# ZulutionAI/MoviiGen1.1

Measured on AMD Instinct MI355X. Metric: denoise-steps/sec, higher is better.
Workload: dtype bf16; 1 GPU; 14B T2V 1920x832x81f bf16 (the metric's configuration; BASELINE configs[2] shape); layers=40, parallelism=single, solver=unipc, weights=random N(0,0.02) bf16, seed 0

## Files before the change

### include/moviigen_hip.h

```cpp
#ifndef MOVIIGEN_HIP_H
#define MOVIIGEN_HIP_H

#include <stdint.h>

#ifdef __cplusplus
extern "C" {
#endif

#define MG_OK 0
#define MG_ERR_ARG (-1)
#define MG_ERR_SHAPE (-2)
#define MG_ERR_LAUNCH (-3)
#define MG_ERR_UNAVAILABLE (-4)
#define MG_ERR_COMM (-5)

const char* mg_version(void);
int mg_abi_version(void);


int mg_ln_modulate(const float* x, int64_t ldx, int64_t rows, int dim, const float* scale,
                   const float* shift, int add_one, float eps, int round_norm_bf16, void* out,
                   int out_f32, int64_t ldo, void* stream);

int64_t mg_step_resid_partials_bytes(void);
int mg_step_resid_capture_f32(float* r, const float* x, const float* xin, int64_t n, double* stats, double* partials,
                              void* stream);
int mg_resid_ln_modulate_f32(const float* x, int64_t ldx, const float* r, int64_t ldr, int64_t rows, int dim,
                             const float* scale, const float* shift, float eps, float* out, int64_t ldo, void* stream);

int mg_rmsnorm_rope_bf16(const uint16_t* x, int64_t ldx, uint16_t* out, int64_t ldo,
                         int64_t rows, int dim, const float* weight, float eps, int head_dim,
                         const float* rope_cs, int F, int H, int W, int64_t pos0, float out_scale, void* stream);

int mg_pack_kv_bf16(const uint16_t* k, int64_t ldk, const uint16_t* v, int64_t ldv, int64_t L,
                    int heads, int head_dim, uint16_t* kp, uint16_t* vp, void* stream);


enum {
    MG_EPI_BIAS_BF16 = 0,
    MG_EPI_BIAS_GELU_BF16 = 1,
    MG_EPI_GATE_RESID_F32 = 2,
    MG_EPI_BIAS_F32 = 3
};

int mg_gemm_bf16(const uint16_t* A, int64_t lda, const uint16_t* W, int64_t ldw,
                 const float* bias, int64_t M, int N, int K, int epilogue, void* out,
                 int64_t ldo, const float* gate, void* stream);

int mg_quant_mxfp8_rows(const uint16_t* x, int64_t ldx, int64_t rows, int K, uint8_t* q, int64_t ldq,
                        uint8_t* scales, int64_t lds, void* stream);

int mg_gemm_mxfp8(const uint8_t* Aq, int64_t lda, const uint8_t* As, int64_t ldas, const uint8_t* Wq, int64_t ldw,
                  const uint8_t* Ws, int64_t ldws, const float* bias, int64_t M, int N, int K, int epilogue,
                  void* out, int64_t ldo, const float* gate, void* stream);

int mg_ln_modulate_mxfp8(const float* x, int64_t ldx, int64_t rows, int dim, const float* scale, const float* shift,
                         int add_one, float eps, int round_norm_bf16, uint16_t* out, int64_t ldo, uint8_t* q,
                         int64_t ldq, uint8_t* scales, int64_t lds, void* stream);

int mg_gemm_mxfp8_gelu_q(const uint8_t* Aq, int64_t lda, const uint8_t* As, int64_t ldas, const uint8_t* Wq, int64_t ldw,
                         const uint8_t* Ws, int64_t ldws, const float* bias, int64_t M, int N, int K, uint8_t* oq,
                         int64_t ldoq, uint8_t* oscales, int64_t ldos, void* stream);

int64_t mg_attn_workspace_bytes(void);
int mg_attn_fwd_bf16_hd128(const uint16_t* q, int64_t ldq, const uint16_t* kp, const uint16_t* vp,
                           uint16_t* o, int64_t ldo, int64_t Lq, int64_t Lk, int heads, float scale,
                           void* workspace, void* stream);

int mg_attn_fwd_bf16_hd128_lse(const uint16_t* q, int64_t ldq, const uint16_t* kp, const uint16_t* vp,
                               uint16_t* o, int64_t ldo, float* lse, int64_t Lq, int64_t Lk, int heads,
                               float scale, void* workspace, void* stream);

int mg_attn_fwd_bf16_hd128_prescaled(const uint16_t* q, int64_t ldq, const uint16_t* kp, const uint16_t* vp,
                                     uint16_t* o, int64_t ldo, float* lse, int64_t Lq, int64_t Lk, int heads,
                                     int reserve_cus, void* workspace, void* stream);

int mg_gate_residual_f32(float* x, int64_t ldx, const uint16_t* y, int64_t ldy, const float* gate, int64_t rows,
                         int dim, void* stream);


int mg_sp_pack_qkv_bf16(const uint16_t* q, int64_t ldq, const uint16_t* k, int64_t ldk, const uint16_t* v,
                        int64_t ldv, int64_t Lloc, int P, int cols_per_dest, int col0, int w, uint16_t* send,
                        void* stream);

int mg_sp_unpack_o_bf16(const uint16_t* recv, int64_t Lloc, int P, int cols_per_src, int col0, int w, uint16_t* o,
                        int64_t ldo, void* stream);

int mg_sp_copy_blocks_bf16(const uint16_t* src, int64_t s_blk, int64_t s_row, uint16_t* dst, int64_t d_blk,
                           int64_t d_row, int blocks, int64_t rows, int width, void* stream);


int mg_comm_unique_id(void* id128);
int mg_comm_create(const void* id128, int nranks, int rank, void** comm);
int mg_comm_destroy(void* comm);

int mg_sp_all_to_all(void* comm, const void* send, void* recv, int64_t bytes_per_peer, void* stream);

int mg_sp_all_to_all_4d_bf16(void* comm, const uint16_t* x, int64_t ldx, int64_t rows, int heads, int head_dim,
                             int seq_to_head, uint16_t* out, int64_t ldo, uint16_t* workspace, void* stream);

int mg_sp_all_gather(void* comm, const void* send, void* recv, int64_t bytes, void* stream);
int mg_shard_all_gather(void* comm, const void* shard, void* full, int64_t shard_bytes, void* stream);

int mg_attn_merge_f32(float* acc, int64_t lda, float* lse_acc, const uint16_t* part, int64_t ldp,
                      const float* lse_part, uint16_t* out, int64_t ldo, int64_t Lq, int heads, int first,
                      void* stream);

int mg_attn_fwd_bf16_generic(const uint16_t* q, int64_t ldq, const uint16_t* k, int64_t ldk,
                             const uint16_t* v, int64_t ldv, uint16_t* o, int64_t ldo, int64_t Lq,
                             int64_t Lk, int heads, int head_dim, float scale, void* stream);


int mg_sinusoid_embed(const void* t, int t_dtype, int n, int dim, float* out, void* stream);

int mg_gemv_f32(const float* W, const float* bias, const float* x, float* y, int N, int K,
                int silu_in, void* stream);

int mg_add_rows_f32(const float* a, const float* b, float* out, int rows, int dim, int period,
                    void* stream);

int mg_head_gemm_f32(const float* x, int64_t ldx, const float* W, const float* bias, float* out,
                     int64_t M, int N, int K, void* stream);

int mg_patchify_bf16(const float* lat, int C, int F, int H, int W, int ph, int pw,
                     uint16_t* out, int64_t ldo, void* stream);

int mg_unpatchify_f32(const float* tok, int64_t ldt, int C, int F, int Hg, int Wg, int ph, int pw,
                      float* lat, void* stream);

int mg_lincomb4_f32(float* out, int64_t n, const float* x0, float c0, const float* x1, float c1,
                    const float* x2, float c2, const float* x3, float c3, void* stream);

int mg_cfg_combine_f32(float* out, const float* uncond, const float* cond, float guide_scale,
                       int64_t n, void* stream);


int mg_embed_rows_bf16(const uint16_t* table, int64_t vocab, int dim, const int64_t* ids, int n,
                       uint16_t* out, void* stream);

int mg_ew_bf16(const uint16_t* a, const uint16_t* b, uint16_t* out, int64_t n, int mode, void* stream);

int mg_t5_attn_bf16(const uint16_t* q, const uint16_t* k, const uint16_t* v, int64_t ld,
                    const uint16_t* rel_emb, const int* rel_bucket, uint16_t* o, int64_t ldo,
                    int64_t Lq, int64_t Lk, int heads, int head_dim, void* stream);


int mg_vae_conv_f32(const float* x, const float* cache, int tc, int T, int H, int W, int Cin,
                    const float* w, const float* bias, int Cout, int kt, int kh, int kw, int up2,
                    const float* residual, float* out, int mode, void* stream);

int mg_vae_upconv_fold_weights_f32(const float* w, int Cout, int Cin, float* wp, void* stream);
int mg_vae_upconv_phases_f32(const float* x, int T, int H, int W, int Cin, const float* wp, const float* bias, int Cout,
                             float* out, int mode, void* stream);

int mg_vae_conv_cols_f32(const float* x, const float* cache, int tc, int T, int H, int W, int Cin,
                         const float* w, const float* bias, int Cout, int kt, int kh, int kw,
                         const float* residual, float* out, int col0, int cols, int mode, void* stream);
int mg_vae_upconv_phases_cols_f32(const float* x, int T, int H, int W, int Cin, const float* wp, const float* bias, int Cout,
                                  float* out, int col0, int cols, int mode, void* stream);

#define MG_VAE_EXACT 0
#define MG_VAE_BF16X3 1
#define MG_VAE_TILE_128 (1 << 8)
#define MG_VAE_TILE_256 (2 << 8)

int mg_vae_rmsnorm_silu_f32(const float* x, const float* gamma, float* out, int64_t rows, int C,
                            int do_silu, void* stream);

int64_t mg_vae_attn_workspace_floats(int64_t L, int C);
int mg_vae_attn_f32(const float* qkv, float* out, int frames, int64_t L, int C, float* workspace,
                    void* stream);
int mg_vae_attn_rows_f32(const float* q, int64_t ldq, const float* k, const float* v, int64_t ldkv, float* out, int frames,
                         int64_t Lq, int64_t Lk, int C, float* workspace, void* stream);

int mg_vae_latent_in_f32(const float* z, const float* mean, const float* inv_std, int C, int T,
                         int H, int W, float* out, void* stream);
int mg_vae_video_out_f32(const float* x, int C, int T, int H, int W, float* out, int t_off,
                         int T_total, void* stream);

int mg_video_to_u8(const float* video, int T, int H, int W, float lo, float hi, uint8_t* frames,
                   void* stream);

int mg_image_to_u8(const float* image, int H, int W, float lo, float hi, uint8_t* pixels, void* stream);

int mg_video_from_u8(const uint8_t* frames, int T, int H0, int W0, int H, int W, float* video, void* stream);

int mg_mask_from_u8(const uint8_t* mask, int Tm, int H0, int W0, int T, int H, int W, int keep_frames, uint8_t* pm, void* stream);

int mg_mask_to_latent_u8(const uint8_t* pm, int T, int H, int W, int st, int sh, int sw, uint8_t* lm, void* stream);

int mg_masked_renoise_f32(float* latent, const float* z0, const float* noise, const uint8_t* lm, float c0, float c1, int C, int64_t thw,
                          void* stream);

int mg_mask_composite_f32(float* video, const float* src, const uint8_t* pm, int T, int64_t hw, void* stream);

int mg_vae_time_interleave_f32(const float* x, int T, int64_t HW, int C, float* out, void* stream);


int mg_vae_conv_strided_f32(const float* x, const float* cache, int tc, int T, int H, int W, int Cin, const float* w, const float* bias,
                            int Cout, int kt, int kh, int kw, int st, int sh, int sw, int pt0, int ph0, int ph1, int pw0, int pw1,
                            float* out, int mode, void* stream);

int mg_vae_conv_in3_f32(const float* xs, const float* cache, int tc, int T, int H, int W, const float* w, const float* bias, int Cout,
                        float* out, int mode, void* stream);

int mg_vae_video_in_f32(const float* video, int T, int H, int W, int t0, int n, float* out, void* stream);
int mg_vae_latent_out_f32(const float* x, int ldx, const float* mean, const float* inv_std, int C, int T, int H, int W, float* out,
                          void* stream);


int mg_lora_merge(void* w, int w_f32, int64_t ldw, int N, int K, const float* up, int64_t ldu, const float* down, int64_t ldd, int R,
                  void* stream);

#ifdef MG_AB_BUILD
int mg_gemm_set_variant(int variant);

int mg_attn_set_variant(int variant);

void mg_attn_w64_profile(unsigned long long* dev_buf);
void mg_attn_w64_debug(int flags);
void mg_attn_w64_flag_counter(unsigned* dev_counter);
void mg_gemm_debug_profile(unsigned long long* dev_buf);
void mg_gemm5_debug_profile(unsigned long long* dev_buf);
#endif

#ifdef __cplusplus
}
#endif
#endif
```

### moviigen1.1_amd/csrc/attn_hd128.hip

```cpp
#include "common.h"
#include "../../include/moviigen_hip.h"

#define ATT_QB 256

__global__ __launch_bounds__(256) void pack_kv_kernel(const uint16_t* __restrict__ k, int64_t ldk,
                                                      const uint16_t* __restrict__ v, int64_t ldv, int64_t L,
                                                      uint16_t* __restrict__ kp, uint16_t* __restrict__ vp, int nt,
                                                      int korder) {
    __shared__ uint16_t tile[64][128 + 8];
    const int head = blockIdx.y, t = blockIdx.x;
    const int64_t k0 = (int64_t)t * 64;
    const int64_t tbase = ((int64_t)head * nt + t) * 8192;
    if (k) {
#pragma unroll
        for (int i = 0; i < 4; ++i) {
            const int id = threadIdx.x + i * 256;
            const int r = id >> 4, c = id & 15;
            u16x8_t u = {0, 0, 0, 0, 0, 0, 0, 0};
            if (k0 + r < L) u = *(const u16x8_t*)(k + (k0 + r) * ldk + head * 128 + c * 8);
            const int row = korder ? ((r & 32) | ((r & 4) << 2) | ((r & 24) >> 1) | (r & 3)) : r;
            *(u16x8_t*)(kp + tbase + c * 512 + row * 8) = u;
        }
    }
    if (v) {
#pragma unroll
        for (int i = 0; i < 4; ++i) {
            const int id = threadIdx.x + i * 256;
            const int r = id >> 4, c = id & 15;
            u16x8_t u = {0, 0, 0, 0, 0, 0, 0, 0};
            if (k0 + r < L) u = *(const u16x8_t*)(v + (k0 + r) * ldv + head * 128 + c * 8);
            *(u16x8_t*)&tile[r][c * 8] = u;
        }
        __syncthreads();
#pragma unroll
        for (int i = 0; i < 4; ++i) {
            const int id = threadIdx.x + i * 256;
            const int kc = id >> 7, d = id & 127;
            u16x8_t u;
#pragma unroll
            for (int j = 0; j < 8; ++j) u[j] = tile[kc * 8 + j][d];
            *(u16x8_t*)(vp + tbase + kc * 1024 + d * 8) = u;
        }
    }
}

#ifdef MG_AB_BUILD
int mg_attn_w64_launch(const uint16_t* q, int64_t ldq, const uint16_t* kp, const uint16_t* vp, uint16_t* o, int64_t ldo,
                       int64_t Lq, int64_t Lk, int heads, float c_log2, int nqb, float* lse, hipStream_t st);
#endif
int mg_attn_m16_launch(const uint16_t* q, int64_t ldq, const uint16_t* kp, const uint16_t* vp, uint16_t* o, int64_t ldo,
                       int64_t Lq, int64_t Lk, int heads, float c_log2, int prescaled, int nqb, float* lse, int reserve_cus,
                       unsigned* workspace, hipStream_t st);

#ifdef MG_AB_BUILD
static int g_attn_variant = 0;
extern "C" int mg_attn_set_variant(int v) {
    if (v != 0 && v != 3) return MG_ERR_ARG;
    g_attn_variant = v;
    return MG_OK;
}
#else
static constexpr int g_attn_variant = 0;
#endif

extern "C" int mg_pack_kv_bf16(const uint16_t* k, int64_t ldk, const uint16_t* v, int64_t ldv, int64_t L, int heads,
                               int head_dim, uint16_t* kp, uint16_t* vp, void* stream) {
    if ((!k && !v) || (k && !kp) || (v && !vp)) return MG_ERR_ARG;
    if (head_dim != 128 || heads <= 0 || L <= 0 || (k && (ldk & 7)) || (v && (ldv & 7))) return MG_ERR_SHAPE;
    const int nt = (int)((L + 63) / 64);
    hipLaunchKernelGGL(pack_kv_kernel, dim3(nt, heads), dim3(256), 0, (hipStream_t)stream, k, ldk, v, ldv, L, kp, vp,
                       nt, g_attn_variant == 3 ? 0 : 1);
    return mg_check_launch();
}

static int attn_fwd_impl(const uint16_t* q, int64_t ldq, const uint16_t* kp, const uint16_t* vp, uint16_t* o, int64_t ldo,
                         float* lse, int64_t Lq, int64_t Lk, int heads, float scale, int prescaled, int reserve_cus, void* workspace,
                         void* stream) {
    if (!q || !kp || !vp || !o) return MG_ERR_ARG;
    if ((uintptr_t)workspace & 7) return MG_ERR_SHAPE;
    if (Lq < 0 || Lk <= 0 || heads <= 0 || reserve_cus < 0) return MG_ERR_SHAPE;
    if ((ldq & 7) || (ldo & 3)) return MG_ERR_SHAPE;
    if (((uintptr_t)q & 15) || ((uintptr_t)kp & 15) || ((uintptr_t)vp & 15) || ((uintptr_t)o & 7)) return MG_ERR_SHAPE;
    if (Lq == 0) return MG_OK;
    const int64_t nqb64 = (Lq + ATT_QB - 1) / ATT_QB;
    if (nqb64 * heads > 0x7fffffffLL) return MG_ERR_SHAPE;
    const int nqb = (int)nqb64;
    const float c_log2 = scale * 1.4426950408889634f;
    hipStream_t st = (hipStream_t)stream;
#ifdef MG_AB_BUILD
    if (g_attn_variant == 3)
        return mg_attn_w64_launch(q, ldq, kp, vp, o, ldo, Lq, Lk, heads, prescaled ? 1.0f : c_log2, nqb, lse, st);
#endif
    return mg_attn_m16_launch(q, ldq, kp, vp, o, ldo, Lq, Lk, heads, c_log2, prescaled, nqb, lse, reserve_cus, (unsigned*)workspace, st);
}

extern "C" int64_t mg_attn_workspace_bytes(void) { return 256; }

extern "C" int mg_attn_fwd_bf16_hd128_lse(const uint16_t* q, int64_t ldq, const uint16_t* kp, const uint16_t* vp,
                                          uint16_t* o, int64_t ldo, float* lse, int64_t Lq, int64_t Lk, int heads,
                                          float scale, void* workspace, void* stream) {
    return attn_fwd_impl(q, ldq, kp, vp, o, ldo, lse, Lq, Lk, heads, scale, 0, 0, workspace, stream);
}
extern "C" int mg_attn_fwd_bf16_hd128(const uint16_t* q, int64_t ldq, const uint16_t* kp, const uint16_t* vp,
                                      uint16_t* o, int64_t ldo, int64_t Lq, int64_t Lk, int heads, float scale,
                                      void* workspace, void* stream) {
    return attn_fwd_impl(q, ldq, kp, vp, o, ldo, nullptr, Lq, Lk, heads, scale, 0, 0, workspace, stream);
}
extern "C" int mg_attn_fwd_bf16_hd128_prescaled(const uint16_t* q, int64_t ldq, const uint16_t* kp, const uint16_t* vp,
                                                uint16_t* o, int64_t ldo, float* lse, int64_t Lq, int64_t Lk, int heads,
                                                int reserve_cus, void* workspace, void* stream) {
    return attn_fwd_impl(q, ldq, kp, vp, o, ldo, lse, Lq, Lk, heads, 1.0f, 1, reserve_cus, workspace, stream);
}
```

### moviigen1.1_amd/csrc/attn_hd128_m16.hip

```cpp
#include <type_traits>
#include "common.h"
#include "../../include/moviigen_hip.h"

#define M16_THREADS 256
#define M16_QB 256
#define M16_TILE 16384
#define M16_K(slot) ((slot) * M16_TILE)
#define M16_V(slot) (3 * M16_TILE + (slot) * M16_TILE)

MG_DEV bf16x8_t m16_bf(u32x4_t v) { return __builtin_bit_cast(bf16x8_t, v); }
struct M16State {
    f32x4_t ot[8][4];
    f32x4_t st[2][2][4];
    bf16x8_t pf[2][4];
    f32x4_t mq[4];
    float m_run[4], l_run[4];
    float psa[4], psb[4];
    int bad;
};

template <int OFF>
MG_DEV void m16_rd(bf16x8_t& dst, unsigned addr) {
    asm volatile("ds_read_b128 %0, %1 offset:%2" : "=v"(dst) : "v"(addr), "i"(OFF));
}
template <int N>
MG_DEV void m16_wait() {
    asm volatile("s_waitcnt lgkmcnt(%0)" ::"i"(N) : "memory");
}
MG_DEV void m16_mfma_s0(f32x4_t& acc, const bf16x8_t& a, const bf16x8_t& b, const f32x4_t& c) {
    asm volatile("v_mfma_f32_16x16x32_bf16 %0, %1, %2, %3" : "=&v"(acc) : "v"(a), "a"(b), "v"(c));
}
MG_DEV void m16_mfma_s(f32x4_t& acc, const bf16x8_t& a, const bf16x8_t& b) {
    asm volatile("v_mfma_f32_16x16x32_bf16 %0, %1, %2, %0" : "+v"(acc) : "v"(a), "a"(b));
}
MG_DEV void m16_mfma_s_after_valu(f32x4_t& acc, const bf16x8_t& a, const bf16x8_t& b) {
    asm volatile("s_nop 7\n\ts_nop 7\n\tv_mfma_f32_16x16x32_bf16 %0, %1, %2, %0" : "+v"(acc) : "v"(a), "a"(b));
}
constexpr int m16_koff(int i) { return (i >> 2) * 256 + (i & 3) * 4096; }
constexpr int m16_voff(int i) { return i * 256; }

template <int KB>
MG_DEV void m16_softmax_exact(M16State& s, float c) {
#pragma unroll
    for (int n = 0; n < 4; ++n) {
        float tmax = s.st[KB][0][n][0];
#pragma unroll
        for (int r = 1; r < 4; ++r) tmax = fmaxf(tmax, s.st[KB][0][n][r]);
#pragma unroll
        for (int r = 0; r < 4; ++r) tmax = fmaxf(tmax, s.st[KB][1][n][r]);
        tmax = fmaxf(tmax, __shfl_xor(tmax, 16, 64));
        tmax = fmaxf(tmax, __shfl_xor(tmax, 32, 64));
        const float m_new = fmaxf(s.m_run[n], tmax);
        float psum = 0.f;
        float p[8];
#pragma unroll
        for (int r = 0; r < 8; ++r) {
            p[r] = __builtin_amdgcn_exp2f((s.st[KB][r >> 2][n][r & 3] - m_new) * c);
            psum += p[r];
        }
        u32x4_t w;
#pragma unroll
        for (int e = 0; e < 4; ++e) w[e] = pack_bf2(p[2 * e], p[2 * e + 1]);
        s.pf[KB][n] = m16_bf(w);
        const float alpha = __builtin_amdgcn_exp2f((s.m_run[n] - m_new) * c);
        s.l_run[n] = s.l_run[n] * alpha + psum;
#pragma unroll
        for (int d = 0; d < 8; ++d)
#pragma unroll
            for (int e = 0; e < 4; ++e) s.ot[d][n][e] *= alpha;
        s.m_run[n] = m_new;
    }
}

template <int KB>
MG_DEV void m16_softmax_zero(M16State& s, float c) {
#pragma unroll
    for (int n = 0; n < 4; ++n) {
        float psum = 0.f;
        float p[8];
#pragma unroll
        for (int r = 0; r < 8; ++r) {
            p[r] = __builtin_amdgcn_exp2f(s.st[KB][r >> 2][n][r & 3] * c);
            psum += p[r];
        }
        u32x4_t w;
#pragma unroll
        for (int e = 0; e < 4; ++e) w[e] = pack_bf2(p[2 * e], p[2 * e + 1]);
        s.pf[KB][n] = m16_bf(w);
        s.l_run[n] += psum;
    }
}

template <int KB>
MG_DEV void m16_mask_init(M16State& s, int lim, int G, const f32x4_t (&base)[4]) {
#pragma unroll
    for (int blk = 0; blk < 2; ++blk)
#pragma unroll
        for (int n = 0; n < 4; ++n)
#pragma unroll
            for (int r = 0; r < 4; ++r) {
                const int key = KB * 32 + G * 8 + blk * 4 + r;
                s.st[KB][blk][n][r] = key >= lim ? -1e30f : base[n][0];
            }
}

template <int KB, int SMODE, bool PV, bool SM, bool SCALED, int ORD, int LKO = 0, int LVO = 0, int NKO = 0, int NVO = 0, typename Dma>
MG_DEV void m16_step(M16State& s, const bf16x8_t (&qf)[4][4], bf16x8_t (&kf)[4], bf16x8_t (&vf)[4], unsigned lds_k,
                     unsigned lds_v, unsigned nk, unsigned nv, float c, Dma dma) {
    constexpr int SB = 1 - KB;
    u32x4_t w[4];
    float pa[2] = {0.f, 0.f}, pb[2] = {0.f, 0.f};
    auto exp_a = [&](int i, int half) __attribute__((always_inline)) {
        if (SM) {
            const int pp = 2 * i + half, n = pp >> 2, wd = pp & 3;
            const float x = s.st[SB][wd >> 1][n][(wd & 1) * 2];
            pa[half] = __builtin_amdgcn_exp2f(SCALED ? x * c : x);
            asm volatile("" : "+v"(pa[half]));
        }
    };
    auto exp_b = [&](int i, int half) __attribute__((always_inline)) {
        if (SM) {
            const int pp = 2 * i + half, n = pp >> 2, wd = pp & 3;
            const float x = s.st[SB][wd >> 1][n][(wd & 1) * 2 + 1];
            pb[half] = __builtin_amdgcn_exp2f(SCALED ? x * c : x);
            asm volatile("" : "+v"(pb[half]));
        }
    };
    auto add_a = [&](int i, int half) __attribute__((always_inline)) {
        if (SM) {
            const int n = (2 * i + half) >> 2;
            s.psa[n] += pa[half];
            asm volatile("" : "+v"(s.psa[n]));
        }
    };
    auto add_b = [&](int i, int half) __attribute__((always_inline)) {
        if (SM) {
            const int n = (2 * i + half) >> 2;
            s.psb[n] += pb[half];
            asm volatile("" : "+v"(s.psb[n]));
        }
    };
    auto cvt = [&](int i, int half) __attribute__((always_inline)) {
        if (SM) {
            const int pp = 2 * i + half, n = pp >> 2, wd = pp & 3;
            unsigned pk = pack_bf2(pa[half], pb[half]);
            asm volatile("" : "+v"(pk));
            w[n][wd] = pk;
        }
    };
    auto S = [&](int i, int n) __attribute__((always_inline)) {
        const int blk = i >> 2, c = i & 3, r = i & 3;
        if (SMODE == 1 && c == 0) m16_mfma_s0(s.st[KB][blk][n], kf[r], qf[n][c], s.mq[n]);
        else if (SMODE == 2 && c == 0) m16_mfma_s_after_valu(s.st[KB][blk][n], kf[r], qf[n][c]);
        else if (SMODE != 0) m16_mfma_s(s.st[KB][blk][n], kf[r], qf[n][c]);
    };
    auto P = [&](int i, int n) __attribute__((always_inline)) {
        if (PV) s.ot[i][n] = __builtin_amdgcn_mfma_f32_16x16x32_bf16(vf[i & 3], s.pf[KB][n], s.ot[i][n], 0, 0, 0);
    };
    auto rdK = [&](int i) __attribute__((always_inline)) {
        const int r2 = (i + 2) & 3;
        if (SMODE == 0) asm volatile("" ::"v"(kf[r2]));
        if (i < 6) {
            switch (i) {
                case 0: m16_rd<m16_koff(2) + LKO>(kf[r2], lds_k); break;
                case 1: m16_rd<m16_koff(3) + LKO>(kf[r2], lds_k); break;
                case 2: m16_rd<m16_koff(4) + LKO>(kf[r2], lds_k); break;
                case 3: m16_rd<m16_koff(5) + LKO>(kf[r2], lds_k); break;
                case 4: m16_rd<m16_koff(6) + LKO>(kf[r2], lds_k); break;
                default: m16_rd<m16_koff(7) + LKO>(kf[r2], lds_k); break;
            }
        } else if (i == 6) m16_rd<m16_koff(0) + NKO>(kf[r2], nk);
        else m16_rd<m16_koff(1) + NKO>(kf[r2], nk);
    };
    auto rdV = [&](int i) __attribute__((always_inline)) {
        const int r2 = (i + 2) & 3;
        if (i < 6) {
            switch (i) {
                case 0: m16_rd<m16_voff(2) + LVO>(vf[r2], lds_v); break;
                case 1: m16_rd<m16_voff(3) + LVO>(vf[r2], lds_v); break;
                case 2: m16_rd<m16_voff(4) + LVO>(vf[r2], lds_v); break;
                case 3: m16_rd<m16_voff(5) + LVO>(vf[r2], lds_v); break;
                case 4: m16_rd<m16_voff(6) + LVO>(vf[r2], lds_v); break;
                default: m16_rd<m16_voff(7) + LVO>(vf[r2], lds_v); break;
            }
        } else if (i == 6) m16_rd<m16_voff(0) + NVO>(vf[r2], nv);
        else m16_rd<m16_voff(1) + NVO>(vf[r2], nv);
    };
#define M16_SB() __builtin_amdgcn_sched_barrier(0)
#pragma unroll
    for (int i = 0; i < 8; ++i) {
        m16_wait<2>();
        M16_SB();
        if constexpr (ORD == 0) {
            S(i, 0); M16_SB();
            exp_a(i, 0); exp_b(i, 0); M16_SB();
            P(i, 0); M16_SB();
            add_a(i, 0); add_b(i, 0); cvt(i, 0); M16_SB();
            S(i, 1); M16_SB();
            rdK(i); M16_SB();
            P(i, 1); M16_SB();
            rdV(i); M16_SB();
            S(i, 2); M16_SB();
            exp_a(i, 1); exp_b(i, 1); M16_SB();
            P(i, 2); M16_SB();
            add_a(i, 1); add_b(i, 1); cvt(i, 1); M16_SB();
            S(i, 3); M16_SB();
            dma(i); M16_SB();
            P(i, 3); M16_SB();
        } else if constexpr (ORD == 1) {
            S(i, 0); M16_SB();
            exp_a(i, 0); M16_SB();
            P(i, 0); M16_SB();
            exp_b(i, 0); M16_SB();
            S(i, 1); M16_SB();
            add_a(i, 0); add_b(i, 0); cvt(i, 0); M16_SB();
            P(i, 1); M16_SB();
            rdK(i); M16_SB(); rdV(i); M16_SB();
            S(i, 2); M16_SB();
            exp_a(i, 1); M16_SB();
            P(i, 2); M16_SB();
            exp_b(i, 1); M16_SB();
            S(i, 3); M16_SB();
            add_a(i, 1); add_b(i, 1); cvt(i, 1); M16_SB();
            P(i, 3); M16_SB();
            dma(i); M16_SB();
        } else if constexpr (ORD == 2) {
            S(i, 0); M16_SB();
            exp_a(i, 0); M16_SB(); rdK(i); M16_SB();
            P(i, 0); M16_SB();
            exp_b(i, 0); M16_SB(); rdV(i); M16_SB();
            S(i, 1); M16_SB();
            add_a(i, 0); add_b(i, 0); cvt(i, 0); M16_SB();
            P(i, 1); M16_SB();
            S(i, 2); M16_SB();
            exp_a(i, 1); M16_SB();
            P(i, 2); M16_SB();
            exp_b(i, 1); M16_SB();
            S(i, 3); M16_SB();
            add_a(i, 1); add_b(i, 1); cvt(i, 1); M16_SB();
            P(i, 3); M16_SB();
            dma(i); M16_SB();
        } else if constexpr (ORD == 4) {
            S(i, 0); M16_SB();
            exp_a(i, 0); M16_SB();
            P(i, 0); M16_SB();
            exp_b(i, 0); M16_SB();
            S(i, 1); M16_SB();
            add_a(i, 0); add_b(i, 0); M16_SB();
            P(i, 1); M16_SB();
            cvt(i, 0); M16_SB(); rdK(i); M16_SB(); rdV(i); M16_SB();
            S(i, 2); M16_SB();
            exp_a(i, 1); M16_SB();
            P(i, 2); M16_SB();
            exp_b(i, 1); M16_SB();
            S(i, 3); M16_SB();
            add_a(i, 1); add_b(i, 1); M16_SB();
            P(i, 3); M16_SB();
            cvt(i, 1); M16_SB(); dma(i); M16_SB();
        } else if constexpr (ORD == 5) {
            S(i, 0); M16_SB();
            exp_a(i, 0); M16_SB();
            P(i, 0); M16_SB();
            exp_b(i, 0); M16_SB();
            S(i, 1); M16_SB();
            add_a(i, 0); add_b(i, 0); cvt(i, 0); M16_SB();
            P(i, 1); M16_SB();
            rdK(i); M16_SB();
            S(i, 2); M16_SB();
            exp_a(i, 1); M16_SB();
            P(i, 2); M16_SB();
            exp_b(i, 1); M16_SB();
            S(i, 3); M16_SB();
            add_a(i, 1); add_b(i, 1); cvt(i, 1); M16_SB();
            P(i, 3); M16_SB();
            rdV(i); M16_SB(); dma(i); M16_SB();
        } else if constexpr (ORD == 8) {
            S(i, 0); M16_SB();
            exp_a(i, 0); M16_SB();
            S(i, 1); M16_SB();
            exp_b(i, 0); M16_SB();
            P(i, 0); M16_SB();
            add_a(i, 0); add_b(i, 0); cvt(i, 0); M16_SB();
            P(i, 1); M16_SB();
            rdK(i); M16_SB(); rdV(i); M16_SB();
            S(i, 2); M16_SB();
            exp_a(i, 1); M16_SB();
            S(i, 3); M16_SB();
            exp_b(i, 1); M16_SB();
            P(i, 2); M16_SB();
            add_a(i, 1); add_b(i, 1); cvt(i, 1); M16_SB();
            P(i, 3); M16_SB();
            dma(i); M16_SB();
        } else if constexpr (ORD == 9) {
            S(i, 0); M16_SB();
            exp_a(i, 0); M16_SB();
            S(i, 1); M16_SB();
            exp_b(i, 0); M16_SB();
            S(i, 2); M16_SB();
            add_a(i, 0); add_b(i, 0); cvt(i, 0); M16_SB();
            S(i, 3); M16_SB();
            rdK(i); M16_SB(); rdV(i); M16_SB();
            P(i, 0); M16_SB();
            exp_a(i, 1); M16_SB();
            P(i, 1); M16_SB();
            exp_b(i, 1); M16_SB();
            P(i, 2); M16_SB();
            add_a(i, 1); add_b(i, 1); cvt(i, 1); M16_SB();
            P(i, 3); M16_SB();
            dma(i); M16_SB();
        } else {
            S(i, 0); M16_SB();
            exp_a(i, 0); M16_SB();
            P(i, 0); M16_SB();
            exp_b(i, 0); M16_SB();
            S(i, 1); M16_SB();
            exp_a(i, 1); M16_SB();
            P(i, 1); M16_SB();
            exp_b(i, 1); M16_SB();
            S(i, 2); M16_SB();
            add_a(i, 0); add_b(i, 0); cvt(i, 0); M16_SB();
            P(i, 2); M16_SB();
            add_a(i, 1); add_b(i, 1); cvt(i, 1); M16_SB();
            S(i, 3); M16_SB();
            rdK(i); M16_SB(); rdV(i); M16_SB();
            P(i, 3); M16_SB();
            dma(i); M16_SB();
        }
    }
#undef M16_SB
    if (SM) {
#pragma unroll
        for (int n = 0; n < 4; ++n) {
            s.pf[SB][n] = m16_bf(w[n]);
        }
    }
}

MG_DEV int m16_lane() {
    int l;
    asm volatile("v_mbcnt_lo_u32_b32 %0, -1, 0\n\tv_mbcnt_hi_u32_b32 %0, -1, %0" : "=v"(l));
    return l;
}

struct M16NoDma {
    __device__ __forceinline__ void operator()(int) const {}
};

template <bool PROF, bool SCALED, int ORD>
__global__ __launch_bounds__(M16_THREADS, 1) void attn_hd128_m16_kernel(
    const uint16_t* __restrict__ q, int64_t ldq, const uint16_t* __restrict__ kp, const uint16_t* __restrict__ vp,
    uint16_t* __restrict__ o, int64_t ldo, int64_t Lq, int64_t Lk, int heads, float c_log2, int nqb, int dbg,
    unsigned long long* __restrict__ prof, float* __restrict__ lse, unsigned* __restrict__ flagcnt, unsigned* __restrict__ tickets) {
    __shared__ __attribute__((aligned(16))) char smem[6 * M16_TILE];
    __shared__ int s_next_item;
    const int bid = blockIdx.x;
    const unsigned long long r_start = PROF ? __builtin_amdgcn_s_memrealtime() : 0;
    const int tid = threadIdx.x;
    const int wave = __builtin_amdgcn_readfirstlane(tid >> 6);
    const int total_items = nqb * heads;
    const int nwg = gridDim.x;
    const bool ticketed = tickets != nullptr && nwg != total_items;
    int item, item_end, item_step;
    if (nwg == total_items || ticketed) {
        item = bid, item_end = ticketed ? total_items : bid + 1, item_step = 1;
    } else {
        const int xcd = bid & 7, slot = bid >> 3;
        item = (int)((int64_t)xcd * total_items / 8) + slot;
        item_end = (int)((int64_t)(xcd + 1) * total_items / 8);
        item_step = nwg >> 3;
    }
    unsigned next_ticket = 0;
    unsigned long long ph[8] = {0, 0, 0, 0, 0, 0, 0, 0}, ph_t = 0;
    unsigned long long pf_fence = 0, pf_a = 0, pf_b = 0, pf_n = 0;
    while (item < item_end) {
    if (ticketed && tid == 0) next_ticket = atomicAdd(tickets, 1u);
    const int head = item / nqb;
    const int qb0 = item - head * nqb;
    const int lane = m16_lane();
    int qi = lane & 15, G = lane >> 4;
    __syncthreads();
    if (PROF) ph_t = __builtin_amdgcn_s_memtime();

    bf16x8_t qf[4][4];
    const int64_t qrow_base = (int64_t)qb0 * M16_QB + wave * 64 + qi;
#pragma unroll
    for (int n = 0; n < 4; ++n) {
        const int64_t qr = qrow_base + n * 16;
        const int64_t qrow = qr < Lq ? qr : Lq - 1;
        const uint16_t* qp = q + qrow * ldq + head * 128 + G * 8;
#pragma unroll
        for (int c = 0; c < 4; ++c) qf[n][c] = m16_bf(*(const u32x4_t*)(qp + c * 32));
    }
    const int T = (int)((Lk + 63) / 64);
    const int last_lim = (int)(Lk - (int64_t)(T - 1) * 64);
    const int nfull = last_lim == 64 ? T : T - 1;
    const unsigned lds0 = (unsigned)(uintptr_t)(mg_lptr_t)smem;
    const uint64_t kb64 = (uint64_t)(uintptr_t)(kp + ((int64_t)head * T) * 8192), vb64 = (uint64_t)(uintptr_t)(vp + ((int64_t)head * T) * 8192);
    const u32x4_t rs_k = {(unsigned)__builtin_amdgcn_readfirstlane((int)(unsigned)kb64), (unsigned)__builtin_amdgcn_readfirstlane((int)((unsigned)(kb64 >> 32) & 0xffffu)),
                          (unsigned)T * M16_TILE, 0x00020000u};
    const u32x4_t rs_v = {(unsigned)__builtin_amdgcn_readfirstlane((int)(unsigned)vb64), (unsigned)__builtin_amdgcn_readfirstlane((int)((unsigned)(vb64 >> 32) & 0xffffu)),
                          (unsigned)T * M16_TILE, 0x00020000u};
    const int dvo = wave * 4096 + lane * 16;
    const unsigned lds_w = (unsigned)__builtin_amdgcn_readfirstlane((int)(lds0 + wave * 4096));
    auto dma_tile4 = [&](const u32x4_t& rs, int t, unsigned lbase) __attribute__((always_inline)) {
        const int soff = __builtin_amdgcn_readfirstlane((t < T ? t : T - 1) * M16_TILE);
        asm volatile("s_mov_b32 m0, %2\n\ts_nop 4\n\t"
                     "buffer_load_dwordx4 %0, %1, %3 offen lds\n\t"
                     "buffer_load_dwordx4 %0, %1, %3 offen offset:1024 lds\n\t"
                     "buffer_load_dwordx4 %0, %1, %3 offen offset:2048 lds\n\t"
                     "buffer_load_dwordx4 %0, %1, %3 offen offset:3072 lds"
                     :: "v"(dvo), "s"(rs), "s"(lbase), "s"(soff) : "memory");
    };
    auto dma_k4 = [&](int t, int slot) __attribute__((always_inline)) { dma_tile4(rs_k, t, lds_w + M16_K(slot)); };
    auto dma_v4 = [&](int t, int slot) __attribute__((always_inline)) { dma_tile4(rs_v, t, lds_w + M16_V(slot)); };
    unsigned kbase = lds0 + G * 1024 + qi * 16;
    unsigned vbase = lds0 + 3 * M16_TILE + G * 2048 + qi * 16;
    auto k_addr = [&](int slot, int kb) __attribute__((always_inline)) { return kbase + slot * M16_TILE + kb * 512; };
    auto v_addr = [&](int slot, int kb) __attribute__((always_inline)) { return vbase + slot * M16_TILE + kb * 8192; };

    M16State s;
    bf16x8_t kf[4], vf[4];
    auto reset = [&]() __attribute__((always_inline)) {
#pragma unroll
        for (int d = 0; d < 8; ++d)
#pragma unroll
            for (int n = 0; n < 4; ++n) s.ot[d][n] = (f32x4_t){0.f, 0.f, 0.f, 0.f};
#pragma unroll
        for (int n = 0; n < 4; ++n) s.m_run[n] = -1e30f, s.l_run[n] = 0.f, s.psa[n] = 0.f, s.psb[n] = 0.f;
        s.bad = 0;
    };
    reset();
    auto q_pin = [&]() __attribute__((always_inline)) {
#pragma unroll
        for (int n = 0; n < 4; ++n)
#pragma unroll
            for (int c = 0; c < 4; ++c) asm volatile("" : "+a"(qf[n][c]));
    };
    auto fence = [&]() __attribute__((always_inline)) {
        asm volatile("s_waitcnt vmcnt(0)" ::: "memory");
        __syncthreads();
    };
    auto fence_hot = [&]() __attribute__((always_inline)) {
        asm volatile("s_waitcnt vmcnt(0)\n\ts_barrier" ::: "memory");
    };
    auto prefetch = [&](unsigned ak, unsigned av) __attribute__((always_inline)) {
        m16_rd<m16_koff(0)>(kf[0], ak);
        m16_rd<m16_voff(0)>(vf[0], av);
        m16_rd<m16_koff(1)>(kf[1], ak);
        m16_rd<m16_voff(1)>(vf[1], av);
    };
    const f32x4_t zero4[4] = {{0.f, 0.f, 0.f, 0.f}, {0.f, 0.f, 0.f, 0.f}, {0.f, 0.f, 0.f, 0.f}, {0.f, 0.f, 0.f, 0.f}};
    auto bare_S = [&](auto kbc, int slot, int lim) __attribute__((always_inline)) {
        constexpr int KB = decltype(kbc)::value;
        if (lim < 64) m16_mask_init<KB>(s, lim, G, zero4);
        else {
#pragma unroll
            for (int blk = 0; blk < 2; ++blk)
#pragma unroll
                for (int n = 0; n < 4; ++n) s.st[KB][blk][n] = (f32x4_t){0.f, 0.f, 0.f, 0.f};
        }
        const char* base = smem + M16_K(slot) + G * 1024 + qi * 16 + KB * 512;
#pragma unroll
        for (int i = 0; i < 8; ++i) {
            const bf16x8_t f = *(const bf16x8_t*)(base + m16_koff(i));
#pragma unroll
            for (int n = 0; n < 4; ++n)
                s.st[KB][i >> 2][n] = __builtin_amdgcn_mfma_f32_16x16x32_bf16(f, qf[n][i & 3], s.st[KB][i >> 2][n], 0, 0, 0);
        }
    };
    auto bare_PV = [&](auto kbc, int slot) __attribute__((always_inline)) {
        constexpr int KB = decltype(kbc)::value;
        const char* base = smem + M16_V(slot) + G * 2048 + qi * 16 + KB * 8192;
#pragma unroll
        for (int i = 0; i < 8; ++i) {
            const bf16x8_t f = *(const bf16x8_t*)(base + m16_voff(i));
#pragma unroll
            for (int n = 0; n < 4; ++n)
                s.ot[i][n] = __builtin_amdgcn_mfma_f32_16x16x32_bf16(f, s.pf[KB][n], s.ot[i][n], 0, 0, 0);
        }
    };
    using KB0 = std::integral_constant<int, 0>;
    using KB1 = std::integral_constant<int, 1>;

    bool exact_pass = nfull < 3;
    if (!exact_pass) {
    for (int attempt = 0;; ++attempt) {
        auto tile_max = [&](float (&mx)[4]) __attribute__((always_inline)) {
#pragma unroll
            for (int n = 0; n < 4; ++n) {
                float a = fmaxf(fmaxf(s.st[0][0][n][0], s.st[0][0][n][1]), fmaxf(s.st[0][0][n][2], s.st[0][0][n][3]));
                float b = fmaxf(fmaxf(s.st[0][1][n][0], s.st[0][1][n][1]), fmaxf(s.st[0][1][n][2], s.st[0][1][n][3]));
                float c2 = fmaxf(fmaxf(s.st[1][0][n][0], s.st[1][0][n][1]), fmaxf(s.st[1][0][n][2], s.st[1][0][n][3]));
                float d2 = fmaxf(fmaxf(s.st[1][1][n][0], s.st[1][1][n][1]), fmaxf(s.st[1][1][n][2], s.st[1][1][n][3]));
                mx[n] = fmaxf(mx[n], fmaxf(fmaxf(a, b), fmaxf(c2, d2)));
            }
        };
        auto set_reference = [&](const float (&mx)[4], float above) __attribute__((always_inline)) {
#pragma unroll
            for (int n = 0; n < 4; ++n) {
                float m = fmaxf(mx[n], __shfl_xor(mx[n], 16, 64));
                m = fmaxf(m, __shfl_xor(m, 32, 64)) + above;
                s.mq[n] = (f32x4_t){-m, -m, -m, -m};
            }
        };
        if (attempt) {
            float mx[4] = {-1e30f, -1e30f, -1e30f, -1e30f};
#pragma unroll
            for (int a = 0; a < 4; ++a) dma_k4(a, a);
            for (int t = 0; t < T; ++t) {
                asm volatile("s_waitcnt vmcnt(12)" ::: "memory");
                __syncthreads();
                dma_k4(t + 4, (t + 4) % 6);
                const int lim = t == T - 1 ? last_lim : 64;
                bare_S(KB0{}, t % 6, lim);
                bare_S(KB1{}, t % 6, lim);
                tile_max(mx);
            }
            asm volatile("s_waitcnt vmcnt(0)" ::: "memory");
            set_reference(mx, 0.f);
            __syncthreads();
            reset();
        }
        dma_k4(0, 0), dma_v4(0, 0), dma_k4(1, 1);
        fence();
        q_pin();
        if (PROF) { const unsigned long long tt = __builtin_amdgcn_s_memtime(); ph[0] += tt - ph_t; ph_t = tt; }
        dma_k4(2, 2), dma_v4(1, 1);
        bare_S(KB0{}, 0, 64);
        bare_S(KB1{}, 0, 64);
        if (attempt == 0) {
            float mx[4] = {-1e30f, -1e30f, -1e30f, -1e30f};
            tile_max(mx);
            set_reference(mx, c_log2 > 1e-20f ? 64.f / c_log2 : 0.f);
        }
#pragma unroll
        for (int kb = 0; kb < 2; ++kb)
#pragma unroll
            for (int blk = 0; blk < 2; ++blk)
#pragma unroll
                for (int n = 0; n < 4; ++n) s.st[kb][blk][n] += s.mq[n];
        m16_softmax_zero<0>(s, c_log2);
#pragma unroll
        for (int n = 0; n < 4; ++n) asm volatile("" : "+v"(s.l_run[n]));
        prefetch(k_addr(1, 0), v_addr(0, 0));
        m16_step<0, 1, true, true, SCALED, ORD>(s, qf, kf, vf, k_addr(1, 0), v_addr(0, 0), k_addr(1, 1), v_addr(0, 1), c_log2, M16NoDma());
        int t = 1;
        unsigned ka0 = k_addr(0, 0), ka1 = k_addr(1, 0), ka2 = k_addr(2, 0);
        unsigned va0 = v_addr(0, 0), va1 = v_addr(1, 0), va2 = v_addr(2, 0);
        unsigned lk0 = (unsigned)__builtin_amdgcn_readfirstlane((int)(lds0 + M16_K(0) + wave * 4096));
        unsigned lk1 = lk0 + M16_TILE, lk2 = lk0 + 2 * M16_TILE;
        int offk = (t + 2) * M16_TILE, offv = (t + 1) * M16_TILE;
        unsigned keep_m0, rot_tmp;
#define M16_BDMA0(VOFF, RS, SOFF, LBASE, IMM)                                                                                              \
    asm volatile("s_add_u32 m0, %2, %3\n\ts_nop 0\n\tbuffer_load_dwordx4 %0, %1, %4 offen lds"                                             \
                 :: "v"(VOFF), "s"(RS), "s"(LBASE), "n"(IMM), "s"(SOFF) : "memory", "scc")
#define M16_BDMAN(VOFF, RS, SOFF, IMM)                                                                                                     \
    asm volatile("buffer_load_dwordx4 %0, %1, %3 offen offset:%2 lds" :: "v"(VOFF), "s"(RS), "n"(IMM), "s"(SOFF) : "memory")
        asm volatile("s_mov_b32 %0, m0\n\ts_nop 4" : "=s"(keep_m0) :: "memory");
        if (PROF) { const unsigned long long tt = __builtin_amdgcn_s_memtime(); ph[1] += tt - ph_t; ph_t = tt; }
        __builtin_amdgcn_s_waitcnt(0x0F70);
        asm volatile("" : "+v"(ka0), "+v"(ka1), "+v"(ka2), "+v"(va0), "+v"(va1), "+v"(va2));
        if (PROF) { const unsigned long long tt = __builtin_amdgcn_s_memtime(); ph[2] += tt - ph_t; ph_t = tt; }
        for (; t + 1 < nfull; ++t) {
            const unsigned long long c0 = PROF ? __builtin_amdgcn_s_memtime() : 0;
            fence_hot();
            const unsigned long long c1 = PROF ? __builtin_amdgcn_s_memtime() : 0;
            m16_step<1, 1, true, true, SCALED, ORD, 512, 8192, 0, 0>(s, qf, kf, vf, ka1, va0, ka2, va1, c_log2,
                                       [&](int n) __attribute__((always_inline)) {
                                           switch (n) {
                                               case 0: M16_BDMA0(dvo, rs_k, offk, lk0, 0); break;
                                               case 1: M16_BDMAN(dvo, rs_k, offk, 1024); break;
                                               case 2: M16_BDMAN(dvo, rs_k, offk, 2048); break;
                                               case 3: M16_BDMAN(dvo, rs_k, offk, 3072); break;
                                               case 4: M16_BDMA0(dvo, rs_v, offv, lk2, 3 * M16_TILE); break;
                                               case 5: M16_BDMAN(dvo, rs_v, offv, 1024); break;
                                               case 6: M16_BDMAN(dvo, rs_v, offv, 2048); break;
                                               default: M16_BDMAN(dvo, rs_v, offv, 3072); break;
                                           }
                                       });
            const unsigned long long c2 = PROF ? __builtin_amdgcn_s_memtime() : 0;
            m16_step<0, 1, true, true, SCALED, ORD, 0, 0, 512, 8192>(s, qf, kf, vf, ka2, va1, ka2, va1, c_log2,
                                       [&](int n) __attribute__((always_inline)) {
                                           if (n == 0)
                                               asm volatile("s_add_u32 %0, %0, 0x4000\n\ts_add_u32 %1, %1, 0x4000" : "+s"(offk), "+s"(offv) : : "scc");
                                           else if (n == 1)
                                               asm volatile("s_mov_b32 %3, %0\n\ts_mov_b32 %0, %1\n\ts_mov_b32 %1, %2\n\ts_mov_b32 %2, %3"
                                                            : "+s"(lk0), "+s"(lk1), "+s"(lk2), "=&s"(rot_tmp));
                                           else if (n == 7) {
                                               asm volatile("v_swap_b32 %0, %1\n\tv_swap_b32 %1, %2" : "+v"(ka0), "+v"(ka1), "+v"(ka2));
                                               asm volatile("v_swap_b32 %0, %1\n\tv_swap_b32 %1, %2" : "+v"(va0), "+v"(va1), "+v"(va2));
                                           }
                                       });
            if (PROF) {
                const unsigned long long c3 = __builtin_amdgcn_s_memtime();
                pf_fence += c1 - c0, pf_a += c2 - c1, pf_b += c3 - c2, pf_n += 1;
            }
        }
#undef M16_BDMA0
#undef M16_BDMAN
        asm volatile("s_mov_b32 m0, %0" :: "s"(keep_m0) : "memory");
        if (PROF) { const unsigned long long tt = __builtin_amdgcn_s_memtime(); ph[3] += tt - ph_t; ph_t = tt; }
        static_assert(M16_TILE == 0x4000, "the literal above");
        const int s0 = (t - 1) % 3, s1 = t % 3, s2 = (t + 1) % 3;
        {
            const int l2 = m16_lane();
            qi = l2 & 15, G = l2 >> 4;
            kbase = lds0 + G * 1024 + qi * 16;
            vbase = lds0 + 3 * M16_TILE + G * 2048 + qi * 16;
        }
        fence();
        if (t + 1 < T) {
            dma_v4(t + 1, s2);
        }
        m16_step<1, 1, true, true, SCALED, ORD>(s, qf, kf, vf, k_addr(s1, 1), v_addr(s0, 1), k_addr(s2, 0), v_addr(s1, 0), c_log2, M16NoDma());
        if (t + 1 < T) {
            m16_mask_init<0>(s, last_lim, G, s.mq);
            m16_step<0, 2, true, true, SCALED, ORD>(s, qf, kf, vf, k_addr(s2, 0), v_addr(s1, 0), k_addr(s2, 1), v_addr(s1, 1), c_log2, M16NoDma());
            fence();
            m16_mask_init<1>(s, last_lim, G, s.mq);
            m16_step<1, 2, true, true, SCALED, ORD>(s, qf, kf, vf, k_addr(s2, 1), v_addr(s1, 1), k_addr(s2, 1), v_addr(s2, 0), c_log2, M16NoDma());
            m16_step<0, 0, true, true, SCALED, ORD>(s, qf, kf, vf, k_addr(s2, 1), v_addr(s2, 0), k_addr(s2, 1), v_addr(s2, 1), c_log2, M16NoDma());
            m16_step<1, 0, true, false, SCALED, ORD>(s, qf, kf, vf, k_addr(s2, 1), v_addr(s2, 1), k_addr(s2, 1), v_addr(s2, 1), c_log2, M16NoDma());
        } else {
            m16_step<0, 0, true, true, SCALED, ORD>(s, qf, kf, vf, k_addr(s1, 1), v_addr(s1, 0), k_addr(s1, 1), v_addr(s1, 1), c_log2, M16NoDma());
            m16_step<1, 0, true, false, SCALED, ORD>(s, qf, kf, vf, k_addr(s1, 1), v_addr(s1, 1), k_addr(s1, 1), v_addr(s1, 1), c_log2, M16NoDma());
        }
        m16_wait<0>();
        asm volatile("" ::"v"(kf[0]), "v"(kf[1]), "v"(kf[2]), "v"(kf[3]), "v"(vf[0]), "v"(vf[1]), "v"(vf[2]), "v"(vf[3]));
#pragma unroll
        for (int n = 0; n < 4; ++n) {
            s.l_run[n] += s.psa[n] + s.psb[n];
            s.psa[n] = s.psb[n] = 0.f;
            float lt = s.l_run[n] + __shfl_xor(s.l_run[n], 16, 64);
            lt += __shfl_xor(lt, 32, 64);
            s.bad |= !(lt >= 8.4703295e-22f && lt <= 1.2379400e27f);
            s.m_run[n] = -s.mq[n][0];
        }
        const bool flagged = __syncthreads_or(s.bad) != 0;
        if (PROF) { const unsigned long long tt = __builtin_amdgcn_s_memtime(); ph[4] += tt - ph_t; ph_t = tt; }
        if (!flagged || (dbg & 1)) break;
        if (flagcnt && tid == 0) atomicAdd(flagcnt + (attempt ? 1 : 0), 1u);
        if (attempt) {
            exact_pass = true;
            break;
        }
    }
    }
    if (exact_pass) {
        reset();
        for (int t = 0; t < T; ++t) {
            __syncthreads();
            dma_k4(t, 0), dma_v4(t, 0);
            fence();
            q_pin();
            const int lim = t == T - 1 ? last_lim : 64;
            bare_S(KB0{}, 0, lim);
            bare_S(KB1{}, 0, lim);
            m16_softmax_exact<0>(s, c_log2);
            bare_PV(KB0{}, 0);
            m16_softmax_exact<1>(s, c_log2);
            bare_PV(KB1{}, 0);
        }
    }

    {
        const int l3 = m16_lane();
        qi = l3 & 15, G = l3 >> 4;
    }
#pragma unroll
    for (int n = 0; n < 4; ++n) {
        float l_tot = s.l_run[n] + __shfl_xor(s.l_run[n], 16, 64);
        l_tot += __shfl_xor(l_tot, 32, 64);
        const float inv = 1.f / l_tot;
        const int64_t qr = (int64_t)qb0 * M16_QB + wave * 64 + n * 16 + qi;
        if (lse && G == 0 && qr < Lq) lse[(int64_t)head * Lq + qr] = (s.m_run[n] * c_log2 + __log2f(l_tot)) * 0.6931471805599453f;
        if (qr < Lq) {
            uint16_t* op = o + qr * ldo + head * 128 + G * 4;
#pragma unroll
            for (int d = 0; d < 8; ++d) {
                uint2 pk;
                pk.x = pack_bf2(s.ot[d][n][0] * inv, s.ot[d][n][1] * inv);
                pk.y = pack_bf2(s.ot[d][n][2] * inv, s.ot[d][n][3] * inv);
                *(uint2*)(op + d * 16) = pk;
            }
        }
    }
    if (PROF) { ph[7] += __builtin_amdgcn_s_memtime() - ph_t; asm volatile("s_waitcnt vmcnt(0)" ::: "memory"); const unsigned long long tt = __builtin_amdgcn_s_memtime(); ph[5] += tt - ph_t; ph[6] += 1; }
    if (ticketed) {
        if (tid == 0) s_next_item = nwg + (int)next_ticket;
        __syncthreads();
        item = __builtin_amdgcn_readfirstlane(s_next_item);
    } else
        item += item_step;
    }
    if (ticketed && tid == 0 && atomicAdd(tickets + 1, 1u) == (unsigned)nwg - 1) {
        __hip_atomic_store(tickets, 0u, __ATOMIC_RELAXED, __HIP_MEMORY_SCOPE_AGENT);
        __hip_atomic_store(tickets + 1, 0u, __ATOMIC_RELAXED, __HIP_MEMORY_SCOPE_AGENT);
    }
    if (PROF && prof && tid == 0) prof[16 + 2 * bid] = r_start, prof[16 + 2 * bid + 1] = __builtin_amdgcn_s_memrealtime();
    if (PROF && prof && (tid & 63) == 0) {
        atomicAdd(prof + wave * 4 + 0, pf_fence);
        atomicAdd(prof + wave * 4 + 1, pf_a);
        atomicAdd(prof + wave * 4 + 2, pf_b);
        atomicAdd(prof + wave * 4 + 3, pf_n);
    }
    if (PROF && prof && tid == 0) {
#pragma unroll
        for (int i = 0; i < 8; ++i) atomicAdd(prof + 1040 + i, ph[i]);
    }
}

static int g_m16_dbg = 0;
static unsigned long long* g_m16_prof = nullptr;
static unsigned* g_m16_flagcnt = nullptr;
void mg_attn_m16_hooks(int dbg, unsigned long long* prof, unsigned* flagcnt) { g_m16_dbg = dbg, g_m16_prof = prof, g_m16_flagcnt = flagcnt; }

int mg_attn_m16_launch(const uint16_t* q, int64_t ldq, const uint16_t* kp, const uint16_t* vp, uint16_t* o, int64_t ldo,
                       int64_t Lq, int64_t Lk, int heads, float c_log2, int prescaled, int nqb, float* lse, int reserve_cus,
                       unsigned* workspace, hipStream_t st) {
    const int n_cu = mg_persistent_cus(reserve_cus);
    if (n_cu < 0) return MG_ERR_LAUNCH;
    const int total = nqb * heads;
    const unsigned grid = total <= n_cu ? (unsigned)total : (unsigned)n_cu;
    unsigned* tickets = nullptr;
    if (workspace && (int64_t)total >= 32 * (int64_t)grid && !(g_m16_dbg & 16))
        tickets = workspace;
#define M16_ORD 9
#define M16_LAUNCH(PROF, SCALED, ORD)                                                                                             \
    hipLaunchKernelGGL((attn_hd128_m16_kernel<PROF, SCALED, ORD>), dim3(grid), dim3(M16_THREADS), 0, st, q, ldq, kp, vp, o, ldo, Lq, \
                       Lk, heads, prescaled ? 1.0f : c_log2, nqb, g_m16_dbg, PROF ? g_m16_prof : nullptr, lse, g_m16_flagcnt, tickets)
#ifdef MG_AB_BUILD
    const int ord = (g_m16_dbg >> 1) & 7;
    const int mo = (g_m16_dbg >> 5) & 3;
    if (mo && prescaled && !g_m16_prof) {
        if (mo == 1) M16_LAUNCH(false, false, 8);
        else if (mo == 2) M16_LAUNCH(false, false, 9);
        else M16_LAUNCH(false, false, 1);
        return mg_check_launch();
    }
    if (ord && prescaled && !g_m16_prof) {
        if (ord == 1) M16_LAUNCH(false, false, 1);
        else if (ord == 2) M16_LAUNCH(false, false, 2);
        else if (ord == 3) M16_LAUNCH(false, false, 3);
        else if (ord == 4) M16_LAUNCH(false, false, 4);
        else if (ord == 5) M16_LAUNCH(false, false, 5);
        else M16_LAUNCH(false, false, 0);
        return mg_check_launch();
    }
#endif
    if (g_m16_prof) {
        if (prescaled) M16_LAUNCH(true, false, M16_ORD);
        else M16_LAUNCH(true, true, M16_ORD);
    } else {
        if (prescaled) M16_LAUNCH(false, false, M16_ORD);
        else M16_LAUNCH(false, true, M16_ORD);
    }
#undef M16_LAUNCH
    return mg_check_launch();
}
```

### moviigen1.1_amd/wan/backend/lib.py

```python
import ctypes
import os

_HERE = os.path.dirname(os.path.abspath(__file__))
LIB_PATH = os.path.normpath(os.path.join(_HERE, '..', '..', 'lib', 'libmoviigen_hip.so'))
LIB_AB_PATH = os.path.normpath(os.path.join(_HERE, '..', '..', 'lib', 'libmoviigen_hip_ab.so'))

c_i64, c_int, c_f32, c_vp = ctypes.c_int64, ctypes.c_int, ctypes.c_float, ctypes.c_void_p

SIGNATURES = {
    'mg_version': [],
    'mg_abi_version': [],
    'mg_ln_modulate': [c_vp, c_i64, c_i64, c_int, c_vp, c_vp, c_int, c_f32, c_int, c_vp, c_int, c_i64, c_vp],
    'mg_step_resid_partials_bytes': [],
    'mg_step_resid_capture_f32': [c_vp, c_vp, c_vp, c_i64, c_vp, c_vp, c_vp],
    'mg_resid_ln_modulate_f32': [c_vp, c_i64, c_vp, c_i64, c_i64, c_int, c_vp, c_vp, c_f32, c_vp, c_i64, c_vp],
    'mg_rmsnorm_rope_bf16': [c_vp, c_i64, c_vp, c_i64, c_i64, c_int, c_vp, c_f32, c_int, c_vp, c_int, c_int,
                             c_int, c_i64, c_f32, c_vp],
    'mg_pack_kv_bf16': [c_vp, c_i64, c_vp, c_i64, c_i64, c_int, c_int, c_vp, c_vp, c_vp],
    'mg_gemm_bf16': [c_vp, c_i64, c_vp, c_i64, c_vp, c_i64, c_int, c_int, c_int, c_vp, c_i64, c_vp, c_vp],
    'mg_quant_mxfp8_rows': [c_vp, c_i64, c_i64, c_int, c_vp, c_i64, c_vp, c_i64, c_vp],
    'mg_gemm_mxfp8': [c_vp, c_i64, c_vp, c_i64, c_vp, c_i64, c_vp, c_i64, c_vp, c_i64, c_int, c_int, c_int, c_vp, c_i64,
                      c_vp, c_vp],
    'mg_ln_modulate_mxfp8': [c_vp, c_i64, c_i64, c_int, c_vp, c_vp, c_int, c_f32, c_int, c_vp, c_i64, c_vp, c_i64, c_vp, c_i64, c_vp],
    'mg_gemm_mxfp8_gelu_q': [c_vp, c_i64, c_vp, c_i64, c_vp, c_i64, c_vp, c_i64, c_vp, c_i64, c_int, c_int, c_vp, c_i64, c_vp, c_i64,
                             c_vp],
    'mg_attn_workspace_bytes': [],
    'mg_attn_fwd_bf16_hd128': [c_vp, c_i64, c_vp, c_vp, c_vp, c_i64, c_i64, c_i64, c_int, c_f32, c_vp, c_vp],
    'mg_attn_fwd_bf16_hd128_lse': [c_vp, c_i64, c_vp, c_vp, c_vp, c_i64, c_vp, c_i64, c_i64, c_int, c_f32, c_vp, c_vp],
    'mg_attn_fwd_bf16_hd128_prescaled': [c_vp, c_i64, c_vp, c_vp, c_vp, c_i64, c_vp, c_i64, c_i64, c_int, c_int, c_vp, c_vp],
    'mg_attn_merge_f32': [c_vp, c_i64, c_vp, c_vp, c_i64, c_vp, c_vp, c_i64, c_i64, c_int, c_int, c_vp],
    'mg_attn_fwd_bf16_generic': [c_vp, c_i64, c_vp, c_i64, c_vp, c_i64, c_vp, c_i64, c_i64, c_i64, c_int, c_int,
                                 c_f32, c_vp],
    'mg_sinusoid_embed': [c_vp, c_int, c_int, c_int, c_vp, c_vp],
    'mg_gemv_f32': [c_vp, c_vp, c_vp, c_vp, c_int, c_int, c_int, c_vp],
    'mg_add_rows_f32': [c_vp, c_vp, c_vp, c_int, c_int, c_int, c_vp],
    'mg_head_gemm_f32': [c_vp, c_i64, c_vp, c_vp, c_vp, c_i64, c_int, c_int, c_vp],
    'mg_patchify_bf16': [c_vp, c_int, c_int, c_int, c_int, c_int, c_int, c_vp, c_i64, c_vp],
    'mg_unpatchify_f32': [c_vp, c_i64, c_int, c_int, c_int, c_int, c_int, c_int, c_vp, c_vp],
    'mg_lincomb4_f32': [c_vp, c_i64, c_vp, c_f32, c_vp, c_f32, c_vp, c_f32, c_vp, c_f32, c_vp],
    'mg_cfg_combine_f32': [c_vp, c_vp, c_vp, c_f32, c_i64, c_vp],
    'mg_embed_rows_bf16': [c_vp, c_i64, c_int, c_vp, c_int, c_vp, c_vp],
    'mg_ew_bf16': [c_vp, c_vp, c_vp, c_i64, c_int, c_vp],
    'mg_t5_attn_bf16': [c_vp, c_vp, c_vp, c_i64, c_vp, c_vp, c_vp, c_i64, c_i64, c_i64, c_int, c_int, c_vp],
    'mg_vae_conv_f32': [c_vp, c_vp, c_int, c_int, c_int, c_int, c_int, c_vp, c_vp, c_int, c_int, c_int, c_int,
                        c_int, c_vp, c_vp, c_int, c_vp],
    'mg_vae_upconv_fold_weights_f32': [c_vp, c_int, c_int, c_vp, c_vp],
    'mg_vae_upconv_phases_f32': [c_vp, c_int, c_int, c_int, c_int, c_vp, c_vp, c_int, c_vp, c_int, c_vp],
    'mg_vae_conv_cols_f32': [c_vp, c_vp, c_int, c_int, c_int, c_int, c_int, c_vp, c_vp, c_int, c_int, c_int, c_int,
                             c_vp, c_vp, c_int, c_int, c_int, c_vp],
    'mg_vae_upconv_phases_cols_f32': [c_vp, c_int, c_int, c_int, c_int, c_vp, c_vp, c_int, c_vp, c_int, c_int, c_int, c_vp],
    'mg_vae_rmsnorm_silu_f32': [c_vp, c_vp, c_vp, c_i64, c_int, c_int, c_vp],
    'mg_vae_attn_workspace_floats': [c_i64, c_int],
    'mg_vae_attn_f32': [c_vp, c_vp, c_int, c_i64, c_int, c_vp, c_vp],
    'mg_vae_attn_rows_f32': [c_vp, c_i64, c_vp, c_vp, c_i64, c_vp, c_int, c_i64, c_i64, c_int, c_vp, c_vp],
    'mg_vae_latent_in_f32': [c_vp, c_vp, c_vp, c_int, c_int, c_int, c_int, c_vp, c_vp],
    'mg_vae_video_out_f32': [c_vp, c_int, c_int, c_int, c_int, c_vp, c_int, c_int, c_vp],
    'mg_vae_time_interleave_f32': [c_vp, c_int, c_i64, c_int, c_vp, c_vp],
    'mg_vae_conv_strided_f32': [c_vp, c_vp, c_int, c_int, c_int, c_int, c_int, c_vp, c_vp, c_int, c_int, c_int, c_int,
                                c_int, c_int, c_int, c_int, c_int, c_int, c_int, c_int, c_vp, c_int, c_vp],
    'mg_vae_conv_in3_f32': [c_vp, c_vp, c_int, c_int, c_int, c_int, c_vp, c_vp, c_int, c_vp, c_int, c_vp],
    'mg_vae_video_in_f32': [c_vp, c_int, c_int, c_int, c_int, c_int, c_vp, c_vp],
    'mg_vae_latent_out_f32': [c_vp, c_int, c_vp, c_vp, c_int, c_int, c_int, c_int, c_vp, c_vp],
    'mg_video_to_u8': [c_vp, c_int, c_int, c_int, c_f32, c_f32, c_vp, c_vp],
    'mg_video_from_u8': [c_vp, c_int, c_int, c_int, c_int, c_int, c_vp, c_vp],
    'mg_mask_from_u8': [c_vp, c_int, c_int, c_int, c_int, c_int, c_int, c_int, c_vp, c_vp],
    'mg_mask_to_latent_u8': [c_vp, c_int, c_int, c_int, c_int, c_int, c_int, c_vp, c_vp],
    'mg_masked_renoise_f32': [c_vp, c_vp, c_vp, c_vp, c_f32, c_f32, c_int, c_i64, c_vp],
    'mg_mask_composite_f32': [c_vp, c_vp, c_vp, c_int, c_i64, c_vp],
    'mg_lora_merge': [c_vp, c_int, c_i64, c_int, c_int, c_vp, c_i64, c_vp, c_i64, c_int, c_vp],
    'mg_comm_unique_id': [c_vp],
    'mg_comm_create': [c_vp, c_int, c_int, c_vp],
    'mg_comm_destroy': [c_vp],
    'mg_sp_all_to_all': [c_vp, c_vp, c_vp, c_i64, c_vp],
    'mg_sp_all_to_all_4d_bf16': [c_vp, c_vp, c_i64, c_i64, c_int, c_int, c_int, c_vp, c_i64, c_vp, c_vp],
    'mg_sp_all_gather': [c_vp, c_vp, c_vp, c_i64, c_vp],
    'mg_shard_all_gather': [c_vp, c_vp, c_vp, c_i64, c_vp],
    'mg_gate_residual_f32': [c_vp, c_i64, c_vp, c_i64, c_vp, c_i64, c_int, c_vp],
    'mg_image_to_u8': [c_vp, c_int, c_int, c_f32, c_f32, c_vp, c_vp],
    'mg_sp_pack_qkv_bf16': [c_vp, c_i64, c_vp, c_i64, c_vp, c_i64, c_i64, c_int, c_int, c_int, c_int, c_vp, c_vp],
    'mg_sp_copy_blocks_bf16': [c_vp, c_i64, c_i64, c_vp, c_i64, c_i64, c_int, c_i64, c_int, c_vp],
    'mg_sp_unpack_o_bf16': [c_vp, c_i64, c_int, c_int, c_int, c_int, c_vp, c_i64, c_vp],
}
SIGNATURES_AB = {
    'mg_attn_set_variant': [c_int],
    'mg_gemm_set_variant': [c_int],
    'mg_attn_w64_profile': [c_vp],
    'mg_attn_w64_debug': [c_int],
    'mg_attn_w64_flag_counter': [c_vp],
    'mg_gemm_debug_profile': [c_vp],
    'mg_gemm5_debug_profile': [c_vp],
}
_RESTYPE = {'mg_version': ctypes.c_char_p, 'mg_vae_attn_workspace_floats': ctypes.c_int64, 'mg_attn_workspace_bytes': ctypes.c_int64,
            'mg_step_resid_partials_bytes': ctypes.c_int64, 'mg_attn_w64_profile': None,
            'mg_attn_w64_debug': None, 'mg_attn_w64_flag_counter': None, 'mg_gemm_debug_profile': None, 'mg_gemm5_debug_profile': None}
DEFAULT_GEMM_VARIANT = 0

ERRORS = {-1: 'MG_ERR_ARG (null pointer / bad enum)', -2: 'MG_ERR_SHAPE (unsupported shape or alignment)',
          -3: 'MG_ERR_LAUNCH (kernel launch failed)', -4: 'MG_ERR_UNAVAILABLE (librccl could not be bound)',
          -5: 'MG_ERR_COMM (an RCCL call failed)'}

_lib = None
_lib_ab = None
_use_ab = False
DEFAULT_ATTN_VARIANT = 0


class MoviigenHipError(RuntimeError):
    pass


def _open(path, sigs):
    if not os.path.exists(path):
        raise MoviigenHipError(
            f'{path} not found: build it with `python __graft_entry__.py build` '
            '(hipcc --offload-arch=gfx950); there is no CPU/torch fallback for the hot path')
    lib = ctypes.CDLL(path)
    for name, args in sigs.items():
        fn = getattr(lib, name)
        fn.argtypes = args
        fn.restype = _RESTYPE.get(name, ctypes.c_int)
    return lib


def load():
    global _lib
    if _use_ab:
        return load_ab()
    if _lib is None:
        _lib = _open(LIB_PATH, SIGNATURES)
    return _lib


def load_ab():
    global _lib_ab
    if _lib_ab is None:
        _lib_ab = _open(LIB_AB_PATH, {**SIGNATURES, **SIGNATURES_AB})
    return _lib_ab


class ab_library:

    def __enter__(self):
        global _use_ab
        self._prev, _use_ab = _use_ab, True
        return load_ab()

    def __exit__(self, *exc):
        global _use_ab
        if self._prev:
            return False
        h = load_ab()
        h.mg_attn_set_variant(DEFAULT_ATTN_VARIANT)
        h.mg_gemm_set_variant(DEFAULT_GEMM_VARIANT)
        h.mg_attn_w64_debug(0)
        h.mg_attn_w64_profile(None)
        h.mg_attn_w64_flag_counter(None)
        h.mg_gemm_debug_profile(None)
        h.mg_gemm5_debug_profile(None)
        _use_ab = self._prev
        return False


def call(name, *args):
    rc = getattr(load(), name)(*args)
    if rc != 0:
        raise MoviigenHipError(f'{name} failed: {ERRORS.get(rc, rc)}')
```

### moviigen1.1_amd/wan/backend/ops.py

```python
import ctypes

import torch

from . import lib

BIAS_BF16, BIAS_GELU_BF16, GATE_RESID_F32, BIAS_F32 = 0, 1, 2, 3


def _p(t):
    return None if t is None else ctypes.c_void_p(t.data_ptr())


def _st():
    return ctypes.c_void_p(torch.cuda.current_stream().cuda_stream)


def _epilogue_dtype(epilogue):
    return torch.bfloat16 if epilogue in (BIAS_BF16, BIAS_GELU_BF16) else torch.float32


def _chk(t, dtype, name):
    if t is None:
        return
    if not t.is_cuda:
        raise lib.MoviigenHipError(f'{name}: expected a CUDA (HIP) tensor — the hot path has no CPU fallback')
    if t.dtype != dtype:
        raise lib.MoviigenHipError(f'{name}: expected {dtype}, got {t.dtype}')
    if t.dim() >= 1 and t.stride(-1) != 1:
        raise lib.MoviigenHipError(f'{name}: innermost dimension must be contiguous')


def ln_modulate(x, scale, shift, add_one, eps, out, round_norm_bf16=False):
    _chk(x, torch.float32, 'x'); _chk(scale, torch.float32, 'scale'); _chk(shift, torch.float32, 'shift')
    rows, dim = x.shape
    lib.call('mg_ln_modulate', _p(x), x.stride(0), rows, dim, _p(scale), _p(shift), int(add_one), float(eps),
             int(round_norm_bf16), _p(out), int(out.dtype == torch.float32), out.stride(0), _st())
    return out


def resid_ln_modulate(x, r, scale, shift, eps, out):
    _chk(x, torch.float32, 'x'); _chk(r, torch.float32, 'r'); _chk(scale, torch.float32, 'scale'); _chk(shift, torch.float32, 'shift')
    _chk(out, torch.float32, 'out')
    if x.dim() != 2 or tuple(r.shape) != tuple(x.shape) or tuple(out.shape) != tuple(x.shape):
        raise lib.MoviigenHipError(f'resid_ln_modulate shape mismatch x{tuple(x.shape)} r{tuple(r.shape)} out{tuple(out.shape)}')
    rows, dim = x.shape
    for name, t in (('scale', scale), ('shift', shift)):
        if t is not None and t.numel() != dim:
            raise lib.MoviigenHipError(f'resid_ln_modulate: {name} must have {dim} elements, got {t.numel()}')
    lib.call('mg_resid_ln_modulate_f32', _p(x), x.stride(0), _p(r), r.stride(0), rows, dim, _p(scale), _p(shift), float(eps), _p(out),
             out.stride(0), _st())
    return out


def step_resid_partials(device):
    return torch.empty(int(lib.load().mg_step_resid_partials_bytes()) // 8, dtype=torch.float64, device=device)


def step_resid_capture(r, x, xin, stats=None, partials=None):
    for name, t in (('r', r), ('x', x), ('xin', xin)):
        _chk(t, torch.float32, name)
        if t is None or not t.is_contiguous():
            raise lib.MoviigenHipError(f'{name} must be a contiguous fp32 tensor')
    if x.numel() != r.numel() or xin.numel() != r.numel():
        raise lib.MoviigenHipError(f'step_resid_capture size mismatch r{tuple(r.shape)} x{tuple(x.shape)} xin{tuple(xin.shape)}')
    if stats is not None:
        _chk(stats, torch.float64, 'stats'); _chk(partials, torch.float64, 'partials')
        if stats.numel() < 2 or not stats.is_contiguous() or partials is None or not partials.is_contiguous() \
                or partials.numel() * 8 < int(lib.load().mg_step_resid_partials_bytes()):
            raise lib.MoviigenHipError('step_resid_capture: stats must be fp64 [2] and partials step_resid_partials(device)')
    lib.call('mg_step_resid_capture_f32', _p(r), _p(x), _p(xin), r.numel(), _p(stats), _p(partials) if stats is not None else None, _st())
    return r


ATTN_LOG2E = 1.4426950408889634


def rmsnorm_rope(x, weight, eps, head_dim, out, rope_cs=None, grid=(1, 1, 1), pos0=0, out_scale=1.0):
    _chk(x, torch.bfloat16, 'x'); _chk(out, torch.bfloat16, 'out'); _chk(weight, torch.float32, 'weight')
    rows, dim = x.shape
    lib.call('mg_rmsnorm_rope_bf16', _p(x), x.stride(0), _p(out), out.stride(0), rows, dim, _p(weight), float(eps),
             int(head_dim), _p(rope_cs), int(grid[0]), int(grid[1]), int(grid[2]), int(pos0), float(out_scale), _st())
    return out


def packed_kv_numel(L, heads):
    return heads * ((L + 63) // 64) * 8192


def pack_kv(k, v, heads, kp, vp):
    _chk(k, torch.bfloat16, 'k'); _chk(v, torch.bfloat16, 'v'); _chk(kp, torch.bfloat16, 'kp'); _chk(vp, torch.bfloat16, 'vp')
    ref = k if k is not None else v
    L = ref.shape[0]
    for name, buf in (('kp', kp if k is not None else None), ('vp', vp if v is not None else None)):
        if buf is not None and buf.numel() < packed_kv_numel(L, heads):
            raise lib.MoviigenHipError(f'{name} too small for {L} keys x {heads} heads')
    lib.call('mg_pack_kv_bf16', _p(k), 0 if k is None else k.stride(0), _p(v), 0 if v is None else v.stride(0), L,
             int(heads), 128, _p(kp), _p(vp), _st())


def gemm(a, w, bias, epilogue, out, gate=None):
    _chk(a, torch.bfloat16, 'a'); _chk(w, torch.bfloat16, 'w'); _chk(bias, torch.float32, 'bias')
    _chk(gate, torch.float32, 'gate')
    _chk(out, _epilogue_dtype(epilogue), 'out')
    M, K = a.shape
    N = w.shape[0]
    if w.shape[1] != K or out.shape[0] != M or out.shape[1] != N:
        raise lib.MoviigenHipError(f'gemm shape mismatch a{tuple(a.shape)} w{tuple(w.shape)} out{tuple(out.shape)}')
    lib.call('mg_gemm_bf16', _p(a), a.stride(0), _p(w), w.stride(0), _p(bias), M, N, K, int(epilogue), _p(out),
             out.stride(0), _p(gate), _st())
    return out


def quant_mxfp8(x, q=None, scales=None):
    _chk(x, torch.bfloat16, 'x')
    if x.dim() != 2:
        raise lib.MoviigenHipError(f'quant_mxfp8: expected [rows, K], got {tuple(x.shape)}')
    rows, K = x.shape
    if q is None:
        q = torch.empty(rows, K, dtype=torch.uint8, device=x.device)
    if scales is None:
        scales = torch.empty(rows, K // 32, dtype=torch.uint8, device=x.device)
    _chk(q, torch.uint8, 'q'); _chk(scales, torch.uint8, 'scales')
    if tuple(q.shape) != (rows, K) or tuple(scales.shape) != (rows, K // 32):
        raise lib.MoviigenHipError(f'quant_mxfp8 shape mismatch x{tuple(x.shape)} q{tuple(q.shape)} scales{tuple(scales.shape)}')
    lib.call('mg_quant_mxfp8_rows', _p(x), x.stride(0), rows, K, _p(q), q.stride(0), _p(scales), scales.stride(0), _st())
    return q, scales


def gemm_mxfp8(aq, a_scales, wq, w_scales, bias, epilogue, out, gate=None):
    _chk(aq, torch.uint8, 'aq'); _chk(a_scales, torch.uint8, 'a_scales'); _chk(wq, torch.uint8, 'wq')
    _chk(w_scales, torch.uint8, 'w_scales'); _chk(bias, torch.float32, 'bias'); _chk(gate, torch.float32, 'gate')
    _chk(out, _epilogue_dtype(epilogue), 'out')
    M, K = aq.shape
    N = wq.shape[0]
    if (wq.shape[1] != K or out.shape[0] != M or out.shape[1] != N or tuple(a_scales.shape) != (M, K // 32)
            or tuple(w_scales.shape) != (N, K // 32)):
        raise lib.MoviigenHipError(f'gemm_mxfp8 shape mismatch aq{tuple(aq.shape)} a_scales{tuple(a_scales.shape)} '
                                   f'wq{tuple(wq.shape)} w_scales{tuple(w_scales.shape)} out{tuple(out.shape)}')
    lib.call('mg_gemm_mxfp8', _p(aq), aq.stride(0), _p(a_scales), a_scales.stride(0), _p(wq), wq.stride(0), _p(w_scales),
             w_scales.stride(0), _p(bias), M, N, K, int(epilogue), _p(out), out.stride(0), _p(gate), _st())
    return out


def ln_modulate_mxfp8(x, scale, shift, add_one, eps, q, scales, out=None, round_norm_bf16=False):
    _chk(x, torch.float32, 'x'); _chk(scale, torch.float32, 'scale'); _chk(shift, torch.float32, 'shift')
    _chk(q, torch.uint8, 'q'); _chk(scales, torch.uint8, 'scales'); _chk(out, torch.bfloat16, 'out')
    rows, dim = x.shape
    if tuple(q.shape) != (rows, dim) or tuple(scales.shape) != (rows, dim // 32) or (out is not None and tuple(out.shape) != (rows, dim)):
        raise lib.MoviigenHipError(f'ln_modulate_mxfp8 shape mismatch x{tuple(x.shape)} q{tuple(q.shape)} scales{tuple(scales.shape)}')
    lib.call('mg_ln_modulate_mxfp8', _p(x), x.stride(0), rows, dim, _p(scale), _p(shift), int(add_one), float(eps),
             int(round_norm_bf16), _p(out), 0 if out is None else out.stride(0), _p(q), q.stride(0), _p(scales), scales.stride(0), _st())
    return q, scales


def gemm_mxfp8_gelu_q(aq, a_scales, wq, w_scales, bias, oq, o_scales):
    _chk(aq, torch.uint8, 'aq'); _chk(a_scales, torch.uint8, 'a_scales'); _chk(wq, torch.uint8, 'wq')
    _chk(w_scales, torch.uint8, 'w_scales'); _chk(bias, torch.float32, 'bias'); _chk(oq, torch.uint8, 'oq')
    _chk(o_scales, torch.uint8, 'o_scales')
    M, K = aq.shape
    N = wq.shape[0]
    if (wq.shape[1] != K or tuple(oq.shape) != (M, N) or tuple(o_scales.shape) != (M, N // 32)
            or tuple(a_scales.shape) != (M, K // 32) or tuple(w_scales.shape) != (N, K // 32)):
        raise lib.MoviigenHipError(f'gemm_mxfp8_gelu_q shape mismatch aq{tuple(aq.shape)} a_scales{tuple(a_scales.shape)} '
                                   f'wq{tuple(wq.shape)} w_scales{tuple(w_scales.shape)} oq{tuple(oq.shape)} o_scales{tuple(o_scales.shape)}')
    lib.call('mg_gemm_mxfp8_gelu_q', _p(aq), aq.stride(0), _p(a_scales), a_scales.stride(0), _p(wq), wq.stride(0), _p(w_scales),
             w_scales.stride(0), _p(bias), M, N, K, _p(oq), oq.stride(0), _p(o_scales), o_scales.stride(0), _st())
    return oq, o_scales


_ATTN_WS = {}


def attention_workspace(device=None, stream=None):
    dev = torch.cuda.current_device() if device is None else torch.device(device).index
    st = torch.cuda.current_stream(dev) if stream is None else stream
    key = (dev, st.cuda_stream)
    ws = _ATTN_WS.get(key)
    if ws is None:
        with torch.cuda.stream(st):
            ws = torch.zeros(int(lib.load().mg_attn_workspace_bytes()), dtype=torch.uint8, device=f'cuda:{dev}')
        _ATTN_WS[key] = ws
    return ws


def attention_hd128(q, kp, vp, out, lk, heads, scale, prescaled=False, reserve_cus=0, workspace='stream', lse=None):
    _chk(q, torch.bfloat16, 'q'); _chk(kp, torch.bfloat16, 'kp'); _chk(vp, torch.bfloat16, 'vp')
    _chk(out, torch.bfloat16, 'out'); _chk(lse, torch.float32, 'lse')
    if min(kp.numel(), vp.numel()) < packed_kv_numel(int(lk), int(heads)):
        raise lib.MoviigenHipError('packed K/V buffers too small for lk keys')
    if lse is not None and (lse.numel() < int(heads) * q.shape[0] or not lse.is_contiguous()):
        raise lib.MoviigenHipError('lse must be a contiguous [heads, Lq] fp32 tensor')
    ws = attention_workspace(q.device) if isinstance(workspace, str) else workspace
    head = (_p(q), q.stride(0), _p(kp), _p(vp), _p(out), out.stride(0))
    if prescaled:
        lib.call('mg_attn_fwd_bf16_hd128_prescaled', *head, _p(lse), q.shape[0], int(lk), int(heads), int(reserve_cus), _p(ws), _st())
    elif lse is not None:
        lib.call('mg_attn_fwd_bf16_hd128_lse', *head, _p(lse), q.shape[0], int(lk), int(heads), float(scale), _p(ws), _st())
    else:
        lib.call('mg_attn_fwd_bf16_hd128', *head, q.shape[0], int(lk), int(heads), float(scale), _p(ws), _st())
    return out


_attention_hd128 = attention_hd128


def attention_hd128_lse(q, kp, vp, out, lse, lk, heads, scale, prescaled=False):
    return _attention_hd128(q, kp, vp, out, lk, heads, scale, prescaled=prescaled, lse=lse), lse


def attention_generic(q, k, v, out, lk, heads, head_dim, scale):
    _chk(q, torch.bfloat16, 'q'); _chk(k, torch.bfloat16, 'k'); _chk(v, torch.bfloat16, 'v')
    _chk(out, torch.bfloat16, 'out')
    lib.call('mg_attn_fwd_bf16_generic', _p(q), q.stride(0), _p(k), k.stride(0), _p(v), v.stride(0), _p(out),
             out.stride(0), q.shape[0], int(lk), int(heads), int(head_dim), float(scale), _st())
    return out


def sinusoid_embed(t, dim, out):
    code = {torch.int64: 0, torch.float32: 1, torch.float64: 2}.get(t.dtype)
    if code is None or not t.is_cuda:
        raise lib.MoviigenHipError('timestep must be a CUDA int64/float32/float64 tensor')
    lib.call('mg_sinusoid_embed', _p(t), code, t.numel(), int(dim), _p(out), _st())
    return out


def gemv(w, bias, x, y, silu_in=False):
    _chk(w, torch.float32, 'w'); _chk(x, torch.float32, 'x'); _chk(y, torch.float32, 'y')
    lib.call('mg_gemv_f32', _p(w), _p(bias), _p(x), _p(y), w.shape[0], w.shape[1], int(silu_in), _st())
    return y


def add_rows(a, b, out, period):
    rows, dim = a.shape
    lib.call('mg_add_rows_f32', _p(a), _p(b), _p(out), rows, dim, int(period), _st())
    return out


def head_gemm(x, w, bias, out):
    _chk(x, torch.float32, 'x'); _chk(w, torch.float32, 'w'); _chk(out, torch.float32, 'out')
    lib.call('mg_head_gemm_f32', _p(x), x.stride(0), _p(w), _p(bias), _p(out), x.shape[0], w.shape[0], w.shape[1],
             _st())
    return out


def patchify(lat, ph, pw, out):
    _chk(lat, torch.float32, 'lat'); _chk(out, torch.bfloat16, 'out')
    C, F, H, W = lat.shape
    lib.call('mg_patchify_bf16', _p(lat), C, F, H, W, int(ph), int(pw), _p(out), out.stride(0), _st())
    return out


def unpatchify(tok, C, F, Hg, Wg, ph, pw, lat):
    _chk(tok, torch.float32, 'tok'); _chk(lat, torch.float32, 'lat')
    lib.call('mg_unpatchify_f32', _p(tok), tok.stride(0), C, F, Hg, Wg, int(ph), int(pw), _p(lat), _st())
    return lat


def lincomb(out, terms):
    terms = list(terms) + [(None, 0.0)] * (4 - len(terms))
    args = []
    for x, c in terms:
        _chk(x, torch.float32, 'x')
        args += [_p(x), float(c)]
    lib.call('mg_lincomb4_f32', _p(out), out.numel(), *args, _st())
    return out


def lora_merge(w, up, down):
    if not torch.is_tensor(w) or w.dtype not in (torch.bfloat16, torch.float32):
        raise lib.MoviigenHipError(f'w: expected a bf16 or fp32 tensor, got {getattr(w, "dtype", type(w))}')
    _chk(w, w.dtype, 'w'); _chk(up, torch.float32, 'up'); _chk(down, torch.float32, 'down')
    if w.dim() != 2 or up.dim() != 2 or down.dim() != 2 or up.shape[0] != w.shape[0] or down.shape[1] != w.shape[1] \
            or up.shape[1] != down.shape[0]:
        raise lib.MoviigenHipError(f'lora_merge shape mismatch w{tuple(w.shape)} up{tuple(up.shape)} down{tuple(down.shape)}')
    N, K = w.shape
    lib.call('mg_lora_merge', _p(w), int(w.dtype == torch.float32), w.stride(0), N, K, _p(up), up.stride(0), _p(down),
             down.stride(0), up.shape[1], _st())
    return w


def cfg_combine(out, uncond, cond, g):
    _chk(uncond, torch.float32, 'uncond'); _chk(cond, torch.float32, 'cond')
    lib.call('mg_cfg_combine_f32', _p(out), _p(uncond), _p(cond), float(g), out.numel(), _st())
    return out


def embed_rows(table, ids, out):
    _chk(table, torch.bfloat16, 'table'); _chk(ids, torch.int64, 'ids'); _chk(out, torch.bfloat16, 'out')
    lib.call('mg_embed_rows_bf16', _p(table), table.shape[0], table.shape[1], _p(ids), ids.numel(), _p(out), _st())
    return out


def ew_bf16(a, b, out, mode):
    for n, t in (('a', a), ('b', b), ('out', out)):
        _chk(t, torch.bfloat16, n)
        if not t.is_contiguous():
            raise lib.MoviigenHipError(f'{n} must be contiguous')
    lib.call('mg_ew_bf16', _p(a), _p(b), _p(out), out.numel(), int(mode), _st())
    return out


def t5_attention(q, k, v, rel_emb, rel_bucket, out, lk, heads, head_dim):
    _chk(q, torch.bfloat16, 'q'); _chk(k, torch.bfloat16, 'k'); _chk(v, torch.bfloat16, 'v')
    _chk(rel_emb, torch.bfloat16, 'rel_emb'); _chk(rel_bucket, torch.int32, 'rel_bucket'); _chk(out, torch.bfloat16, 'out')
    if not (q.stride(0) == k.stride(0) == v.stride(0)):
        raise lib.MoviigenHipError('q, k, v must share a row stride')
    if rel_bucket.numel() != q.shape[0] + int(lk) - 1:
        raise lib.MoviigenHipError('rel_bucket must have Lq + Lk - 1 entries')
    lib.call('mg_t5_attn_bf16', _p(q), _p(k), _p(v), q.stride(0), _p(rel_emb), _p(rel_bucket), _p(out), out.stride(0),
             q.shape[0], int(lk), int(heads), int(head_dim), _st())
    return out


VAE_EXACT, VAE_BF16X3 = 0, 1


def vae_conv(x, w, bias, out, kt, kh, kw, cache=None, up2=False, residual=None, mode=VAE_EXACT):
    for n, t in (('x', x), ('w', w), ('bias', bias), ('out', out), ('cache', cache), ('residual', residual)):
        _chk(t, torch.float32, n)
    T, H, W, Cin = x.shape
    tc = 0 if cache is None else cache.shape[0]
    lib.call('mg_vae_conv_f32', _p(x), _p(cache), tc, T, H, W, Cin, _p(w), _p(bias), w.shape[0], kt, kh, kw,
             int(up2), _p(residual), _p(out), int(mode), _st())
    return out


def vae_conv_cols(x, w, bias, out, kt, kh, kw, col0, cache=None, residual=None, mode=VAE_EXACT):
    for n, t in (('x', x), ('w', w), ('bias', bias), ('out', out), ('cache', cache), ('residual', residual)):
        _chk(t, torch.float32, n)
    T, H, W, Cin = x.shape
    cols = out.shape[2]
    if out.shape[0] != T or out.shape[1] != H or not out.is_contiguous() or not x.is_contiguous():
        raise lib.MoviigenHipError(f'vae_conv_cols: out {tuple(out.shape)} does not match x {tuple(x.shape)}')
    if cache is not None and (tuple(cache.shape[1:]) != tuple(x.shape[1:]) or not cache.is_contiguous()):
        raise lib.MoviigenHipError('vae_conv_cols: the cache must have the haloed geometry of x')
    tc = 0 if cache is None else cache.shape[0]
    lib.call('mg_vae_conv_cols_f32', _p(x), _p(cache), tc, T, H, W, Cin, _p(w), _p(bias), w.shape[0], kt, kh, kw,
             _p(residual), _p(out), int(col0), int(cols), int(mode), _st())
    return out


def vae_upconv_fold_weights(w):
    _chk(w, torch.float32, 'w')
    Cout, kt, kh, kw, Cin = w.shape
    if (kt, kh, kw) != (1, 3, 3):
        raise ValueError(f'the phase decomposition is defined for 1x3x3 kernels, got {kt}x{kh}x{kw}')
    wp = torch.empty(4, Cout, 2, 2, Cin, dtype=torch.float32, device=w.device)
    lib.call('mg_vae_upconv_fold_weights_f32', _p(w), Cout, Cin, _p(wp), _st())
    return wp


def vae_upconv_phases(x, wp, bias, out, mode=VAE_EXACT):
    for n, t in (('x', x), ('wp', wp), ('bias', bias), ('out', out)):
        _chk(t, torch.float32, n)
    T, H, W, Cin = x.shape
    lib.call('mg_vae_upconv_phases_f32', _p(x), T, H, W, Cin, _p(wp), _p(bias), wp.shape[1], _p(out), int(mode), _st())
    return out


def vae_upconv_phases_cols(x, wp, bias, out, col0, mode=VAE_EXACT):
    for n, t in (('x', x), ('wp', wp), ('bias', bias), ('out', out)):
        _chk(t, torch.float32, n)
    T, H, W, Cin = x.shape
    if out.shape[0] != T or out.shape[1] != 2 * H or out.shape[2] % 2 or not out.is_contiguous() or not x.is_contiguous():
        raise lib.MoviigenHipError(f'vae_upconv_phases_cols: out {tuple(out.shape)} does not match x {tuple(x.shape)}')
    lib.call('mg_vae_upconv_phases_cols_f32', _p(x), T, H, W, Cin, _p(wp), _p(bias), wp.shape[1], _p(out), int(col0), out.shape[2] // 2,
             int(mode), _st())
    return out


def vae_rmsnorm_silu(x, gamma, out, do_silu=True):
    C = x.shape[-1]
    lib.call('mg_vae_rmsnorm_silu_f32', _p(x), _p(gamma), _p(out), x.numel() // C, C, int(do_silu), _st())
    return out


def vae_attn_workspace_floats(L, C):
    return int(lib.load().mg_vae_attn_workspace_floats(int(L), int(C)))


def vae_attn(qkv, out, workspace):
    frames, L, C3 = qkv.shape
    if workspace.numel() < vae_attn_workspace_floats(L, C3 // 3):
        raise lib.MoviigenHipError('vae_attn workspace too small')
    lib.call('mg_vae_attn_f32', _p(qkv), _p(out), frames, L, C3 // 3, _p(workspace), _st())
    return out


def vae_attn_rows(q, kv, out, workspace):
    for n, t in (('q', q), ('kv', kv), ('out', out), ('workspace', workspace)):
        _chk(t, torch.float32, n)
    frames, Lq = q.shape[:2]
    Lk, C = kv.shape[1], kv.shape[2] // 2
    if kv.shape[0] != frames or not kv.is_contiguous() or not out.is_contiguous() or q.stride(0) != Lq * q.stride(1) or out.shape != (frames, Lq, C):
        raise lib.MoviigenHipError('vae_attn_rows: shapes')
    if workspace.numel() < vae_attn_workspace_floats(Lk, C):
        raise lib.MoviigenHipError('vae_attn workspace too small')
    lib.call('mg_vae_attn_rows_f32', _p(q), q.stride(1), _p(kv), ctypes.c_void_p(kv.data_ptr() + 4 * C), 2 * C, _p(out), frames, Lq, Lk, C,
             _p(workspace), _st())
    return out


def vae_latent_in(z, mean, inv_std, out):
    C, T, H, W = z.shape
    lib.call('mg_vae_latent_in_f32', _p(z), _p(mean), _p(inv_std), C, T, H, W, _p(out), _st())
    return out


def vae_video_out(x, out, t_off):
    T, H, W, C = x.shape
    lib.call('mg_vae_video_out_f32', _p(x), C, T, H, W, _p(out), int(t_off), out.shape[1], _st())
    return out


def vae_time_interleave(x, out):
    T, H, W, C2 = x.shape
    lib.call('mg_vae_time_interleave_f32', _p(x), T, H * W, C2 // 2, _p(out), _st())
    return out


def vae_conv_strided_out_shape(x_shape, kernel, stride, pad_t0, pad_h, pad_w):
    T, H, W = x_shape[:3]
    (kt, kh, kw), (st, sh, sw) = kernel, stride
    return [(T + pad_t0 - kt) // st + 1, (H + pad_h[0] + pad_h[1] - kh) // sh + 1, (W + pad_w[0] + pad_w[1] - kw) // sw + 1]


def vae_conv_strided(x, w, bias, out, stride, pad_t0=0, pad_h=(0, 0), pad_w=(0, 0), cache=None, mode=VAE_EXACT):
    for n, t in (('x', x), ('w', w), ('bias', bias), ('out', out), ('cache', cache)):
        _chk(t, torch.float32, n)
    T, H, W, Cin = x.shape
    Cout, kt, kh, kw, wc = w.shape
    want = vae_conv_strided_out_shape(x.shape, (kt, kh, kw), stride, pad_t0, pad_h, pad_w) + [Cout]
    if wc != Cin or list(out.shape) != want or not out.is_contiguous() or not x.is_contiguous() or not w.is_contiguous():
        raise lib.MoviigenHipError(f'vae_conv_strided: x {tuple(x.shape)}, w {tuple(w.shape)} need a contiguous out {want}, got {tuple(out.shape)}')
    if cache is not None and (tuple(cache.shape[1:]) != tuple(x.shape[1:]) or not cache.is_contiguous()):
        raise lib.MoviigenHipError('vae_conv_strided: the cache must have the frame geometry of x')
    tc = 0 if cache is None else cache.shape[0]
    lib.call('mg_vae_conv_strided_f32', _p(x), _p(cache), tc, T, H, W, Cin, _p(w), _p(bias), Cout, kt, kh, kw, int(stride[0]), int(stride[1]),
             int(stride[2]), int(pad_t0), int(pad_h[0]), int(pad_h[1]), int(pad_w[0]), int(pad_w[1]), _p(out), int(mode), _st())
    return out


def vae_video_in(video, t0, n, out):
    _chk(video, torch.float32, 'video'); _chk(out, torch.float32, 'out')
    if video.dim() != 4 or video.shape[0] != 3 or not video.is_contiguous():
        raise lib.MoviigenHipError('video must be a contiguous [3, T, H, W] tensor')
    _, T, H, W = video.shape
    if tuple(out.shape) != (n, H, W + 2, 4) or not out.is_contiguous():
        raise lib.MoviigenHipError(f'vae_video_in: out must be a contiguous {(n, H, W + 2, 4)} tensor, got {tuple(out.shape)}')
    lib.call('mg_vae_video_in_f32', _p(video), T, H, W, int(t0), int(n), _p(out), _st())
    return out


def vae_conv_in3(xs, w, bias, out, cache=None, mode=VAE_EXACT):
    for n, t in (('xs', xs), ('w', w), ('bias', bias), ('out', out), ('cache', cache)):
        _chk(t, torch.float32, n)
    T, H, Wp, c4 = xs.shape
    Cout = w.shape[0]
    if c4 != 4 or tuple(w.shape) != (Cout, 3, 3, 3, 4) or tuple(out.shape) != (T, H, Wp - 2, Cout) or not (xs.is_contiguous() and w.is_contiguous()
                                                                                                     and out.is_contiguous()):
        raise lib.MoviigenHipError(f'vae_conv_in3: xs {tuple(xs.shape)}, w {tuple(w.shape)}, out {tuple(out.shape)}')
    if cache is not None and (tuple(cache.shape[1:]) != tuple(xs.shape[1:]) or not cache.is_contiguous()):
        raise lib.MoviigenHipError('vae_conv_in3: the cache must have the staged frame geometry of xs')
    tc = 0 if cache is None else cache.shape[0]
    lib.call('mg_vae_conv_in3_f32', _p(xs), _p(cache), tc, T, H, Wp - 2, _p(w), _p(bias), Cout, _p(out), int(mode), _st())
    return out


def vae_latent_out(x, mean, inv_std, out):
    for n, t in (('x', x), ('mean', mean), ('inv_std', inv_std), ('out', out)):
        _chk(t, torch.float32, n)
    T, H, W, Cx = x.shape
    C = out.shape[0]
    if tuple(out.shape) != (C, T, H, W) or C > Cx or mean.numel() < C or inv_std.numel() < C or not (x.is_contiguous() and out.is_contiguous()):
        raise lib.MoviigenHipError(f'vae_latent_out: x {tuple(x.shape)}, out {tuple(out.shape)}')
    lib.call('mg_vae_latent_out_f32', _p(x), Cx, _p(mean), _p(inv_std), C, T, H, W, _p(out), _st())
    return out


def video_to_u8(video, lo=-1.0, hi=1.0):
    _chk(video, torch.float32, 'video')
    if video.dim() != 4 or video.shape[0] != 3 or not video.is_contiguous():
        raise lib.MoviigenHipError('video must be a contiguous [3, T, H, W] tensor')
    _, T, H, W = video.shape
    out = torch.empty(T, H, W, 3, dtype=torch.uint8, device=video.device)
    lib.call('mg_video_to_u8', _p(video), T, H, W, float(lo), float(hi), _p(out), _st())
    return out


def video_from_u8(frames, H, W, out=None):
    _chk(frames, torch.uint8, 'frames'); _chk(out, torch.float32, 'out')
    if frames.dim() != 4 or frames.shape[3] != 3 or not frames.is_contiguous():
        raise lib.MoviigenHipError(f'frames must be a contiguous uint8 [T, H0, W0, 3] tensor, got {tuple(frames.shape)}')
    T, H0, W0, _ = frames.shape
    if out is None:
        out = torch.empty(3, T, int(H), int(W), dtype=torch.float32, device=frames.device)
    elif tuple(out.shape) != (3, T, int(H), int(W)) or not out.is_contiguous():
        raise lib.MoviigenHipError(f'video_from_u8: out must be a contiguous {(3, T, int(H), int(W))} tensor, got {tuple(out.shape)}')
    lib.call('mg_video_from_u8', _p(frames), T, H0, W0, int(H), int(W), _p(out), _st())
    return out


def mask_from_u8(mask, T, H, W, keep_frames=0, out=None):
    _chk(mask, torch.uint8, 'mask'); _chk(out, torch.uint8, 'out')
    if mask.dim() != 3 or not mask.is_contiguous():
        raise lib.MoviigenHipError(f'mask must be a contiguous uint8 [Tm, H0, W0] tensor, got {tuple(mask.shape)}')
    Tm, H0, W0 = mask.shape
    if out is None:
        out = torch.empty(int(T), int(H), int(W), dtype=torch.uint8, device=mask.device)
    elif tuple(out.shape) != (int(T), int(H), int(W)) or not out.is_contiguous():
        raise lib.MoviigenHipError(f'mask_from_u8: out must be a contiguous {(int(T), int(H), int(W))} tensor, got {tuple(out.shape)}')
    lib.call('mg_mask_from_u8', _p(mask), Tm, H0, W0, int(T), int(H), int(W), int(keep_frames), _p(out), _st())
    return out


def mask_to_latent(pm, stride):
    _chk(pm, torch.uint8, 'pm')
    if pm.dim() != 3 or not pm.is_contiguous():
        raise lib.MoviigenHipError(f'pm must be a contiguous uint8 [T, H, W] tensor, got {tuple(pm.shape)}')
    T, H, W = pm.shape
    st, sh, sw = (int(v) for v in stride)
    if min(st, sh, sw) <= 0:
        raise lib.MoviigenHipError(f'mask_to_latent: stride must be positive, got {(st, sh, sw)}')
    lm = torch.empty((T - 1) // st + 1, H // sh, W // sw, dtype=torch.uint8, device=pm.device)
    lib.call('mg_mask_to_latent_u8', _p(pm), T, H, W, st, sh, sw, _p(lm), _st())
    return lm


def masked_renoise(latent, z0, noise, lm, c0, c1):
    for n, t in (('latent', latent), ('z0', z0), ('noise', noise)):
        _chk(t, torch.float32, n)
    _chk(lm, torch.uint8, 'lm')
    if not (latent.is_contiguous() and z0.is_contiguous() and noise.is_contiguous() and lm.is_contiguous()) or latent.dim() < 2 \
            or z0.shape != latent.shape or noise.shape != latent.shape or lm.numel() * latent.shape[0] != latent.numel():
        raise lib.MoviigenHipError(f'masked_renoise: latent {tuple(latent.shape)}, z0 {tuple(z0.shape)}, noise {tuple(noise.shape)}, lm {tuple(lm.shape)}')
    lib.call('mg_masked_renoise_f32', _p(latent), _p(z0), _p(noise), _p(lm), float(c0), float(c1), latent.shape[0], lm.numel(), _st())
    return latent


def mask_composite(video, src, pm):
    _chk(video, torch.float32, 'video'); _chk(src, torch.float32, 'src'); _chk(pm, torch.uint8, 'pm')
    if video.dim() != 4 or video.shape[0] != 3 or src.shape != video.shape or tuple(pm.shape) != tuple(video.shape[1:]) \
            or not (video.is_contiguous() and src.is_contiguous() and pm.is_contiguous()):
        raise lib.MoviigenHipError(f'mask_composite: video {tuple(video.shape)}, src {tuple(src.shape)}, pm {tuple(pm.shape)}')
    T = video.shape[1]
    lib.call('mg_mask_composite_f32', _p(video), _p(src), _p(pm), T, video.shape[2] * video.shape[3], _st())
    return video


def gate_residual(x, y, gate=None):
    _chk(x, torch.float32, 'x'); _chk(y, torch.bfloat16, 'y'); _chk(gate, torch.float32, 'gate')
    if x.shape != y.shape:
        raise lib.MoviigenHipError(f'gate_residual shape mismatch x{tuple(x.shape)} y{tuple(y.shape)}')
    lib.call('mg_gate_residual_f32', _p(x), x.stride(0), _p(y), y.stride(0), _p(gate), x.shape[0], x.shape[1], _st())
    return x


def sp_pack_qkv(q, k, v, P, cols_per_dest, col0, w, send):
    for n, t in (('q', q), ('k', k), ('v', v), ('send', send)):
        _chk(t, torch.bfloat16, n)
    Lloc = q.shape[0]
    if send.numel() < P * Lloc * 3 * w or not send.is_contiguous():
        raise lib.MoviigenHipError('send buffer too small / not contiguous')
    lib.call('mg_sp_pack_qkv_bf16', _p(q), q.stride(0), _p(k), k.stride(0), _p(v), v.stride(0), Lloc, int(P),
             int(cols_per_dest), int(col0), int(w), _p(send), _st())
    return send


def sp_unpack_o(recv, P, cols_per_src, col0, w, o):
    _chk(recv, torch.bfloat16, 'recv'); _chk(o, torch.bfloat16, 'o')
    Lloc = o.shape[0]
    if recv.numel() < P * Lloc * w or not recv.is_contiguous():
        raise lib.MoviigenHipError('recv buffer too small / not contiguous')
    lib.call('mg_sp_unpack_o_bf16', _p(recv), Lloc, int(P), int(cols_per_src), int(col0), int(w), _p(o), o.stride(0), _st())
    return o


def sp_copy_blocks(src, s_blk, s_row, dst, d_blk, d_row, blocks, rows, width):
    _chk(src, torch.bfloat16, 'src'); _chk(dst, torch.bfloat16, 'dst')
    lib.call('mg_sp_copy_blocks_bf16', _p(src), int(s_blk), int(s_row), _p(dst), int(d_blk), int(d_row), int(blocks),
             int(rows), int(width), _st())
    return dst


def image_to_u8(image, lo=-1.0, hi=1.0):
    _chk(image, torch.float32, 'image')
    if image.dim() != 3 or image.shape[0] != 3 or not image.is_contiguous():
        raise lib.MoviigenHipError('image must be a contiguous [3, H, W] tensor')
    _, H, W = image.shape
    out = torch.empty(H, W, 3, dtype=torch.uint8, device=image.device)
    lib.call('mg_image_to_u8', _p(image), H, W, float(lo), float(hi), _p(out), _st())
    return out


def attention_merge(acc, lse_acc, part, lse_part, heads, first, out=None):
    _chk(acc, torch.float32, 'acc'); _chk(lse_acc, torch.float32, 'lse_acc'); _chk(part, torch.bfloat16, 'part')
    _chk(lse_part, torch.float32, 'lse_part'); _chk(out, torch.bfloat16, 'out')
    lib.call('mg_attn_merge_f32', _p(acc), acc.stride(0), _p(lse_acc), _p(part), part.stride(0), _p(lse_part), _p(out),
             out.stride(0) if out is not None else 0, acc.shape[0], int(heads), int(bool(first)), _st())
    return acc
```

### moviigen1.1_amd/wan/distributed/ulysses.py

```python
import os

import torch

from ..backend import ops
from . import collectives, peer_copy

_a2a = collectives.all_to_all


def split_heads(n_loc, max_groups):
    G = max(1, min(int(n_loc), int(max_groups)))
    base, extra = divmod(n_loc, G)
    out, h0 = [], 0
    for g in range(G):
        n = base + (1 if g < extra else 0)
        out.append((h0, n))
        h0 += n
    return out


def attention_rounds(n_heads, L, n_cu=256, qblock=256):
    items = n_heads * ((L + qblock - 1) // qblock)
    per_xcd_wg = max(1, (n_cu & ~7) // 8)
    if items <= (n_cu & ~7):
        return 1
    return max(((x + 1) * items // 8 - x * items // 8 + per_xcd_wg - 1) // per_xcd_wg for x in range(8))


def choose_groups(n_loc, L, P, dim=None, max_groups=5, n_cu=256, tflops_per_cu=5.8, link_gbps=45.0):
    dim = dim if dim is not None else 128 * n_loc * P
    t_item = 4.0 * 256 * L * 128 / (tflops_per_cu * 1e12) * 1e3
    t_exch = 4.0 * (L / P) * dim * 2 / P / (link_gbps * 1e9) * 1e3 if P > 1 else 0.0
    best = None
    for G in range(1, max(1, min(int(n_loc), int(max_groups))) + 1):
        rounds = sum(attention_rounds(n, L, n_cu) for _, n in split_heads(n_loc, G))
        cost = rounds * t_item + t_exch / G
        if best is None or cost < best[2] - 1e-9 or (abs(cost - best[2]) <= 1e-9 and G > best[0]):
            best = (G, rounds, cost)
    return best


class HeadExchange:

    trace = None

    @classmethod
    def _mark(cls, kind, stream):
        if cls.trace is None:
            return None
        ev = torch.cuda.Event(enable_timing=True)
        ev.record(stream)
        cls.trace.append((kind, ev))
        return ev

    @classmethod
    def overlap_summary(cls):
        s = collectives.trace_summary(cls.trace or [])
        return {'exchange_ms': s['comm_ms'], 'exposed_ms': s['exposed_ms'], 'hidden_frac': s['hidden_frac'], 'collectives': s['collectives']}

    def __init__(self, group, P, heads, head_dim, Lloc, device, max_groups=None):
        if heads % P:
            raise ValueError(f'`num_heads` {heads} cannot be divided evenly by the sequence-parallel size {P}')
        self.group, self.P, self.hd, self.Lloc = group, P, head_dim, Lloc
        self.n_loc = heads // P
        self.cols = self.n_loc * head_dim
        n_cu = torch.cuda.get_device_properties(device).multi_processor_count if torch.device(device).type == 'cuda' else 256
        want_reserve = 0 if peer_copy.wanted(group, device) else (int(os.environ.get('MOVIIGEN_SP_RESERVE_CUS', '0') or 0) + 7) & ~7
        n_cu_attn = max(8, (n_cu & ~7) - want_reserve)
        if max_groups is None:
            env = os.environ.get('MOVIIGEN_SP_GROUPS', '') or 'auto'
            if env == 'auto':
                max_groups = choose_groups(self.n_loc, P * Lloc, P, dim=heads * head_dim, n_cu=n_cu_attn)[0] if head_dim == 128 else min(5, self.n_loc)
            else:
                max_groups = int(env)
        self.groups = split_heads(self.n_loc, max_groups)
        bf = torch.bfloat16
        e = lambda *s: torch.empty(*s, dtype=bf, device=device)
        self.send, self.recv, self.ag, self.orecv = [], [], [], []
        for _, n in self.groups:
            w = n * head_dim
            self.send.append(e(P, Lloc, 3 * w))
            self.recv.append(e(P * Lloc, 3 * w))
            self.ag.append(e(P * Lloc, w))
            self.orecv.append(e(P, Lloc, w))
        self.peer = None
        if peer_copy.wanted(group, device):
            self.peer = peer_copy.open_windows(group, self.recv + self.orecv)
        self.comm = torch.cuda.Stream(device=device)
        self.reserve_cus = 0 if self.peer is not None or len(self.groups) < 2 else int(os.environ.get('MOVIIGEN_SP_RESERVE_CUS', '0') or 0)
        self.rounds = sum(attention_rounds(n, P * Lloc, (n_cu & ~7) - ((self.reserve_cus + 7) & ~7)) for _, n in self.groups)
        ev = lambda: [torch.cuda.Event() for _ in self.groups]
        self.ev_pack, self.ev_recv, self.ev_attn, self.ev_o = ev(), ev(), ev(), ev()

    def peer_failed(self):
        return self.peer is not None and self.peer.failed()

    def drop_peer(self):
        import logging
        if self.peer is not None:
            logging.warning('Ulysses exchange: the peer-copy transport reported a failed copy; this exchange now uses the all-to-all collective')
        self.peer = None
        self.reserve_cus = 0 if len(self.groups) < 2 else int(os.environ.get('MOVIIGEN_SP_RESERVE_CUS', '0') or 0)

    def run(self, q, k, v, out, attend):
        P, hd, cur = self.P, self.hd, torch.cuda.current_stream()
        for g, (h0, n) in enumerate(self.groups):
            ops.sp_pack_qkv(q, k, v, P, self.cols, h0 * hd, n * hd, self.send[g])
            self.ev_pack[g].record(cur)
        with torch.cuda.stream(self.comm):
            for g in range(len(self.groups)):
                self.comm.wait_event(self.ev_pack[g])
                self._mark('comm', self.comm)
                if self.peer is not None:
                    self.peer.all_to_all(g, self.send[g])
                else:
                    _a2a(self.recv[g].view(P, self.Lloc, -1), self.send[g], self.group)
                self._mark('comm', self.comm)
                self.ev_recv[g].record(self.comm)
        for g, (h0, n) in enumerate(self.groups):
            w = n * hd
            self._mark('wait', cur)
            cur.wait_event(self.ev_recv[g])
            self._mark('wait', cur)
            r = self.recv[g]
            attend(r[:, :w], r[:, w:2 * w], r[:, 2 * w:], self.ag[g], n)
            self.ev_attn[g].record(cur)
            with torch.cuda.stream(self.comm):
                self.comm.wait_event(self.ev_attn[g])
                self._mark('comm', self.comm)
                if self.peer is not None:
                    self.peer.all_to_all(len(self.groups) + g, self.ag[g].view(P, self.Lloc, w))
                else:
                    _a2a(self.orecv[g], self.ag[g].view(P, self.Lloc, w), self.group)
                self._mark('comm', self.comm)
                self.ev_o[g].record(self.comm)
        for g, (h0, n) in enumerate(self.groups):
            self._mark('wait', cur)
            cur.wait_event(self.ev_o[g])
            self._mark('wait', cur)
            ops.sp_unpack_o(self.orecv[g], P, self.cols, h0 * hd, n * hd, out)
        return out


def seq_to_head(x, out, group, P, heads, head_dim):
    Lloc = x.shape[0]
    nl = (heads // P) * head_dim
    if x.is_cuda:
        send = torch.empty(P, Lloc, nl, dtype=x.dtype, device=x.device)
        ops.sp_copy_blocks(x, nl, x.stride(0), send, Lloc * nl, nl, P, Lloc, nl)
    else:
        send = x.reshape(Lloc, P, nl).transpose(0, 1).contiguous()
    _a2a(out.view(P, Lloc, nl), send, group)
    return out


def head_to_seq(x, out, group, P, heads, head_dim):
    nl = (heads // P) * head_dim
    Lloc = x.shape[0] // P
    recv = torch.empty(P, Lloc, nl, dtype=x.dtype, device=x.device)
    _a2a(recv, x.view(P, Lloc, nl), group)
    if x.is_cuda:
        ops.sp_copy_blocks(recv, Lloc * nl, nl, out, nl, out.stride(0), P, Lloc, nl)
    else:
        out.view(Lloc, P, nl).copy_(recv.transpose(0, 1))
    return out


def all_gather_seq(x, group, P):
    out = torch.empty(P * x.shape[0], x.shape[1], dtype=x.dtype, device=x.device)
    collectives.all_gather(out, x.contiguous(), group)
    return out
```

Baseline: 0.04646 steps/s.

## Add five-block query tiles to hd128 attention with cost-based tile selection

Templates the m16 flash-attention kernel on the number of 16-row query blocks per wave and adds a 5-block (320 queries per workgroup) variant with its own interleaved MFMA/exp schedule. A host-side cost model picks 320 or 256 queries per item for long prescaled sequences, and the Ulysses group planner uses the same model. The intent is to reuse each K/V fragment read from LDS across more queries and to cut the number of work items. The cost is higher register pressure and a new schedule that has to stay correct for tail blocks.

Result: faster. 0.04740 steps/s, median of 6 (+2.0%).

```diff
diff --git a/include/moviigen_hip.h b/include/moviigen_hip.h
--- a/include/moviigen_hip.h
+++ b/include/moviigen_hip.h
@@ -63,6 +63,7 @@
                          int64_t ldoq, uint8_t* oscales, int64_t ldos, void* stream);
 
 int64_t mg_attn_workspace_bytes(void);
+int mg_attn_hd128_item_queries(int64_t Lq, int64_t Lk, int heads, int prescaled, int n_cu);
 int mg_attn_fwd_bf16_hd128(const uint16_t* q, int64_t ldq, const uint16_t* kp, const uint16_t* vp,
                            uint16_t* o, int64_t ldo, int64_t Lq, int64_t Lk, int heads, float scale,
                            void* workspace, void* stream);
diff --git a/moviigen1.1_amd/csrc/attn_hd128.hip b/moviigen1.1_amd/csrc/attn_hd128.hip
--- a/moviigen1.1_amd/csrc/attn_hd128.hip
+++ b/moviigen1.1_amd/csrc/attn_hd128.hip
@@ -49,7 +49,7 @@
                        int64_t Lq, int64_t Lk, int heads, float c_log2, int nqb, float* lse, hipStream_t st);
 #endif
 int mg_attn_m16_launch(const uint16_t* q, int64_t ldq, const uint16_t* kp, const uint16_t* vp, uint16_t* o, int64_t ldo,
-                       int64_t Lq, int64_t Lk, int heads, float c_log2, int prescaled, int nqb, float* lse, int reserve_cus,
+                       int64_t Lq, int64_t Lk, int heads, float c_log2, int prescaled, float* lse, int reserve_cus,
                        unsigned* workspace, hipStream_t st);
 
 #ifdef MG_AB_BUILD
@@ -84,14 +84,13 @@
     if (Lq == 0) return MG_OK;
     const int64_t nqb64 = (Lq + ATT_QB - 1) / ATT_QB;
     if (nqb64 * heads > 0x7fffffffLL) return MG_ERR_SHAPE;
-    const int nqb = (int)nqb64;
     const float c_log2 = scale * 1.4426950408889634f;
     hipStream_t st = (hipStream_t)stream;
 #ifdef MG_AB_BUILD
     if (g_attn_variant == 3)
-        return mg_attn_w64_launch(q, ldq, kp, vp, o, ldo, Lq, Lk, heads, prescaled ? 1.0f : c_log2, nqb, lse, st);
+        return mg_attn_w64_launch(q, ldq, kp, vp, o, ldo, Lq, Lk, heads, prescaled ? 1.0f : c_log2, (int)nqb64, lse, st);
 #endif
-    return mg_attn_m16_launch(q, ldq, kp, vp, o, ldo, Lq, Lk, heads, c_log2, prescaled, nqb, lse, reserve_cus, (unsigned*)workspace, st);
+    return mg_attn_m16_launch(q, ldq, kp, vp, o, ldo, Lq, Lk, heads, c_log2, prescaled, lse, reserve_cus, (unsigned*)workspace, st);
 }
 
 extern "C" int64_t mg_attn_workspace_bytes(void) { return 256; }
diff --git a/moviigen1.1_amd/csrc/attn_hd128_m16.hip b/moviigen1.1_amd/csrc/attn_hd128_m16.hip
--- a/moviigen1.1_amd/csrc/attn_hd128_m16.hip
+++ b/moviigen1.1_amd/csrc/attn_hd128_m16.hip
@@ -3,19 +3,19 @@
 #include "../../include/moviigen_hip.h"
 
 #define M16_THREADS 256
-#define M16_QB 256
 #define M16_TILE 16384
 #define M16_K(slot) ((slot) * M16_TILE)
 #define M16_V(slot) (3 * M16_TILE + (slot) * M16_TILE)
 
 MG_DEV bf16x8_t m16_bf(u32x4_t v) { return __builtin_bit_cast(bf16x8_t, v); }
+template <int NQ>
 struct M16State {
-    f32x4_t ot[8][4];
-    f32x4_t st[2][2][4];
-    bf16x8_t pf[2][4];
-    f32x4_t mq[4];
-    float m_run[4], l_run[4];
-    float psa[4], psb[4];
+    f32x4_t ot[8][NQ];
+    f32x4_t st[2][2][NQ];
+    bf16x8_t pf[2][NQ];
+    f32x4_t mq[NQ];
+    float m_run[NQ], l_run[NQ];
+    float psa[NQ], psb[NQ];
     int bad;
 };
 
@@ -39,10 +39,10 @@
 constexpr int m16_koff(int i) { return (i >> 2) * 256 + (i & 3) * 4096; }
 constexpr int m16_voff(int i) { return i * 256; }
 
-template <int KB>
-MG_DEV void m16_softmax_exact(M16State& s, float c) {
-#pragma unroll
-    for (int n = 0; n < 4; ++n) {
+template <int KB, int NQ>
+MG_DEV void m16_softmax_exact(M16State<NQ>& s, float c) {
+#pragma unroll
+    for (int n = 0; n < NQ; ++n) {
         float tmax = s.st[KB][0][n][0];
 #pragma unroll
         for (int r = 1; r < 4; ++r) tmax = fmaxf(tmax, s.st[KB][0][n][r]);
@@ -72,10 +72,10 @@
     }
 }
 
-template <int KB>
-MG_DEV void m16_softmax_zero(M16State& s, float c) {
-#pragma unroll
-    for (int n = 0; n < 4; ++n) {
+template <int KB, int NQ>
+MG_DEV void m16_softmax_zero(M16State<NQ>& s, float c) {
+#pragma unroll
+    for (int n = 0; n < NQ; ++n) {
         float psum = 0.f;
         float p[8];
 #pragma unroll
@@ -91,12 +91,12 @@
     }
 }
 
-template <int KB>
-MG_DEV void m16_mask_init(M16State& s, int lim, int G, const f32x4_t (&base)[4]) {
+template <int KB, int NQ>
+MG_DEV void m16_mask_init(M16State<NQ>& s, int lim, int G, const f32x4_t (&base)[NQ]) {
 #pragma unroll
     for (int blk = 0; blk < 2; ++blk)
 #pragma unroll
-        for (int n = 0; n < 4; ++n)
+        for (int n = 0; n < NQ; ++n)
 #pragma unroll
             for (int r = 0; r < 4; ++r) {
                 const int key = KB * 32 + G * 8 + blk * 4 + r;
@@ -104,50 +104,56 @@
             }
 }
 
-template <int KB, int SMODE, bool PV, bool SM, bool SCALED, int ORD, int LKO = 0, int LVO = 0, int NKO = 0, int NVO = 0, typename Dma>
-MG_DEV void m16_step(M16State& s, const bf16x8_t (&qf)[4][4], bf16x8_t (&kf)[4], bf16x8_t (&vf)[4], unsigned lds_k,
+template <int KB, int SMODE, bool PV, bool SM, bool SCALED, int ORD, int NQ, int LKO = 0, int LVO = 0, int NKO = 0, int NVO = 0, typename Dma>
+MG_DEV void m16_step(M16State<NQ>& s, const bf16x8_t (&qf)[NQ][4], bf16x8_t (&kf)[4], bf16x8_t (&vf)[4], unsigned lds_k,
                      unsigned lds_v, unsigned nk, unsigned nv, float c, Dma dma) {
+    static_assert(NQ == 4 || (NQ == 5 && ORD == 9), "the five-block groups exist for the shipped order only");
     constexpr int SB = 1 - KB;
-    u32x4_t w[4];
+    u32x4_t w[NQ];
     float pa[2] = {0.f, 0.f}, pb[2] = {0.f, 0.f};
-    auto exp_a = [&](int i, int half) __attribute__((always_inline)) {
+    auto exp_a_p = [&](int pp, int half) __attribute__((always_inline)) {
         if (SM) {
-            const int pp = 2 * i + half, n = pp >> 2, wd = pp & 3;
+            const int n = pp >> 2, wd = pp & 3;
             const float x = s.st[SB][wd >> 1][n][(wd & 1) * 2];
             pa[half] = __builtin_amdgcn_exp2f(SCALED ? x * c : x);
             asm volatile("" : "+v"(pa[half]));
         }
     };
-    auto exp_b = [&](int i, int half) __attribute__((always_inline)) {
+    auto exp_b_p = [&](int pp, int half) __attribute__((always_inline)) {
         if (SM) {
-            const int pp = 2 * i + half, n = pp >> 2, wd = pp & 3;
+            const int n = pp >> 2, wd = pp & 3;
             const float x = s.st[SB][wd >> 1][n][(wd & 1) * 2 + 1];
             pb[half] = __builtin_amdgcn_exp2f(SCALED ? x * c : x);
             asm volatile("" : "+v"(pb[half]));
         }
     };
-    auto add_a = [&](int i, int half) __attribute__((always_inline)) {
+    auto add_a_p = [&](int pp, int half) __attribute__((always_inline)) {
         if (SM) {
-            const int n = (2 * i + half) >> 2;
+            const int n = pp >> 2;
             s.psa[n] += pa[half];
             asm volatile("" : "+v"(s.psa[n]));
         }
     };
-    auto add_b = [&](int i, int half) __attribute__((always_inline)) {
+    auto add_b_p = [&](int pp, int half) __attribute__((always_inline)) {
         if (SM) {
-            const int n = (2 * i + half) >> 2;
+            const int n = pp >> 2;
             s.psb[n] += pb[half];
             asm volatile("" : "+v"(s.psb[n]));
         }
     };
-    auto cvt = [&](int i, int half) __attribute__((always_inline)) {
+    auto cvt_p = [&](int pp, int half) __attribute__((always_inline)) {
         if (SM) {
-            const int pp = 2 * i + half, n = pp >> 2, wd = pp & 3;
+            const int n = pp >> 2, wd = pp & 3;
             unsigned pk = pack_bf2(pa[half], pb[half]);
             asm volatile("" : "+v"(pk));
             w[n][wd] = pk;
         }
     };
+    auto exp_a = [&](int i, int half) __attribute__((always_inline)) { exp_a_p(2 * i + half, half); };
+    auto exp_b = [&](int i, int half) __attribute__((always_inline)) { exp_b_p(2 * i + half, half); };
+    auto add_a = [&](int i, int half) __attribute__((always_inline)) { add_a_p(2 * i + half, half); };
+    auto add_b = [&](int i, int half) __attribute__((always_inline)) { add_b_p(2 * i + half, half); };
+    auto cvt = [&](int i, int half) __attribute__((always_inline)) { cvt_p(2 * i + half, half); };
     auto S = [&](int i, int n) __attribute__((always_inline)) {
         const int blk = i >> 2, c = i & 3, r = i & 3;
         if (SMODE == 1 && c == 0) m16_mfma_s0(s.st[KB][blk][n], kf[r], qf[n][c], s.mq[n]);
@@ -191,7 +197,53 @@
     for (int i = 0; i < 8; ++i) {
         m16_wait<2>();
         M16_SB();
-        if constexpr (ORD == 0) {
+        if constexpr (NQ == 5) {
+            auto aac = [&](int pp) __attribute__((always_inline)) { add_a_p(pp, pp & 1); add_b_p(pp, pp & 1); cvt_p(pp, pp & 1); };
+            if ((i & 1) == 0) {
+                const int p0 = 5 * i / 2;
+                S(i, 0); M16_SB();
+                exp_a_p(p0, p0 & 1); M16_SB();
+                S(i, 1); M16_SB();
+                exp_b_p(p0, p0 & 1); M16_SB();
+                S(i, 2); M16_SB();
+                aac(p0); M16_SB();
+                S(i, 3); M16_SB();
+                rdK(i); M16_SB(); rdV(i); M16_SB();
+                S(i, 4); M16_SB();
+                exp_a_p(p0 + 1, (p0 + 1) & 1); M16_SB();
+                P(i, 0); M16_SB();
+                exp_b_p(p0 + 1, (p0 + 1) & 1); M16_SB();
+                P(i, 1); M16_SB();
+                aac(p0 + 1); M16_SB();
+                P(i, 2); M16_SB();
+                exp_a_p(p0 + 2, (p0 + 2) & 1); M16_SB();
+                P(i, 3); M16_SB();
+                dma(i); M16_SB();
+                P(i, 4); M16_SB();
+            } else {
+                const int p0 = (5 * i - 1) / 2;
+                S(i, 0); M16_SB();
+                exp_b_p(p0, p0 & 1); M16_SB();
+                S(i, 1); M16_SB();
+                aac(p0); M16_SB();
+                S(i, 2); M16_SB();
+                exp_a_p(p0 + 1, (p0 + 1) & 1); M16_SB();
+                S(i, 3); M16_SB();
+                exp_b_p(p0 + 1, (p0 + 1) & 1); M16_SB();
+                S(i, 4); M16_SB();
+                aac(p0 + 1); M16_SB();
+                P(i, 0); M16_SB();
+                rdK(i); M16_SB(); rdV(i); M16_SB();
+                P(i, 1); M16_SB();
+                exp_a_p(p0 + 2, (p0 + 2) & 1); M16_SB();
+                P(i, 2); M16_SB();
+                exp_b_p(p0 + 2, (p0 + 2) & 1); M16_SB();
+                P(i, 3); M16_SB();
+                aac(p0 + 2); M16_SB();
+                P(i, 4); M16_SB();
+                dma(i); M16_SB();
+            }
+        } else if constexpr (ORD == 0) {
             S(i, 0); M16_SB();
             exp_a(i, 0); exp_b(i, 0); M16_SB();
             P(i, 0); M16_SB();
@@ -330,7 +382,7 @@
 #undef M16_SB
     if (SM) {
 #pragma unroll
-        for (int n = 0; n < 4; ++n) {
+        for (int n = 0; n < NQ; ++n) {
             s.pf[SB][n] = m16_bf(w[n]);
         }
     }
@@ -346,7 +398,7 @@
     __device__ __forceinline__ void operator()(int) const {}
 };
 
-template <bool PROF, bool SCALED, int ORD>
+template <bool PROF, bool SCALED, int ORD, int NQ>
 __global__ __launch_bounds__(M16_THREADS, 1) void attn_hd128_m16_kernel(
     const uint16_t* __restrict__ q, int64_t ldq, const uint16_t* __restrict__ kp, const uint16_t* __restrict__ vp,
     uint16_t* __restrict__ o, int64_t ldo, int64_t Lq, int64_t Lk, int heads, float c_log2, int nqb, int dbg,
@@ -381,10 +433,10 @@
     __syncthreads();
     if (PROF) ph_t = __builtin_amdgcn_s_memtime();
 
-    bf16x8_t qf[4][4];
-    const int64_t qrow_base = (int64_t)qb0 * M16_QB + wave * 64 + qi;
-#pragma unroll
-    for (int n = 0; n < 4; ++n) {
+    bf16x8_t qf[NQ][4];
+    const int64_t qrow_base = (int64_t)qb0 * (64 * NQ) + wave * (16 * NQ) + qi;
+#pragma unroll
+    for (int n = 0; n < NQ; ++n) {
         const int64_t qr = qrow_base + n * 16;
         const int64_t qrow = qr < Lq ? qr : Lq - 1;
         const uint16_t* qp = q + qrow * ldq + head * 128 + G * 8;
@@ -418,21 +470,21 @@
     auto k_addr = [&](int slot, int kb) __attribute__((always_inline)) { return kbase + slot * M16_TILE + kb * 512; };
     auto v_addr = [&](int slot, int kb) __attribute__((always_inline)) { return vbase + slot * M16_TILE + kb * 8192; };
 
-    M16State s;
+    M16State<NQ> s;
     bf16x8_t kf[4], vf[4];
     auto reset = [&]() __attribute__((always_inline)) {
 #pragma unroll
         for (int d = 0; d < 8; ++d)
 #pragma unroll
-            for (int n = 0; n < 4; ++n) s.ot[d][n] = (f32x4_t){0.f, 0.f, 0.f, 0.f};
-#pragma unroll
-        for (int n = 0; n < 4; ++n) s.m_run[n] = -1e30f, s.l_run[n] = 0.f, s.psa[n] = 0.f, s.psb[n] = 0.f;
+            for (int n = 0; n < NQ; ++n) s.ot[d][n] = (f32x4_t){0.f, 0.f, 0.f, 0.f};
+#pragma unroll
+        for (int n = 0; n < NQ; ++n) s.m_run[n] = -1e30f, s.l_run[n] = 0.f, s.psa[n] = 0.f, s.psb[n] = 0.f;
         s.bad = 0;
     };
     reset();
     auto q_pin = [&]() __attribute__((always_inline)) {
 #pragma unroll
-        for (int n = 0; n < 4; ++n)
+        for (int n = 0; n < NQ; ++n)
 #pragma unroll
             for (int c = 0; c < 4; ++c) asm volatile("" : "+a"(qf[n][c]));
     };
@@ -449,7 +501,7 @@
         m16_rd<m16_koff(1)>(kf[1], ak);
         m16_rd<m16_voff(1)>(vf[1], av);
     };
-    const f32x4_t zero4[4] = {{0.f, 0.f, 0.f, 0.f}, {0.f, 0.f, 0.f, 0.f}, {0.f, 0.f, 0.f, 0.f}, {0.f, 0.f, 0.f, 0.f}};
+    const f32x4_t zero4[NQ] = {};
     auto bare_S = [&](auto kbc, int slot, int lim) __attribute__((always_inline)) {
         constexpr int KB = decltype(kbc)::value;
         if (lim < 64) m16_mask_init<KB>(s, lim, G, zero4);
@@ -457,14 +509,14 @@
 #pragma unroll
             for (int blk = 0; blk < 2; ++blk)
 #pragma unroll
-                for (int n = 0; n < 4; ++n) s.st[KB][blk][n] = (f32x4_t){0.f, 0.f, 0.f, 0.f};
+                for (int n = 0; n < NQ; ++n) s.st[KB][blk][n] = (f32x4_t){0.f, 0.f, 0.f, 0.f};
         }
         const char* base = smem + M16_K(slot) + G * 1024 + qi * 16 + KB * 512;
 #pragma unroll
         for (int i = 0; i < 8; ++i) {
             const bf16x8_t f = *(const bf16x8_t*)(base + m16_koff(i));
 #pragma unroll
-            for (int n = 0; n < 4; ++n)
+            for (int n = 0; n < NQ; ++n)
                 s.st[KB][i >> 2][n] = __builtin_amdgcn_mfma_f32_16x16x32_bf16(f, qf[n][i & 3], s.st[KB][i >> 2][n], 0, 0, 0);
         }
     };
@@ -475,7 +527,7 @@
         for (int i = 0; i < 8; ++i) {
             const bf16x8_t f = *(const bf16x8_t*)(base + m16_voff(i));
 #pragma unroll
-            for (int n = 0; n < 4; ++n)
+            for (int n = 0; n < NQ; ++n)
                 s.ot[i][n] = __builtin_amdgcn_mfma_f32_16x16x32_bf16(f, s.pf[KB][n], s.ot[i][n], 0, 0, 0);
         }
     };
@@ -485,9 +537,9 @@
     bool exact_pass = nfull < 3;
     if (!exact_pass) {
     for (int attempt = 0;; ++attempt) {
-        auto tile_max = [&](float (&mx)[4]) __attribute__((always_inline)) {
-#pragma unroll
-            for (int n = 0; n < 4; ++n) {
+        auto tile_max = [&](float (&mx)[NQ]) __attribute__((always_inline)) {
+#pragma unroll
+            for (int n = 0; n < NQ; ++n) {
                 float a = fmaxf(fmaxf(s.st[0][0][n][0], s.st[0][0][n][1]), fmaxf(s.st[0][0][n][2], s.st[0][0][n][3]));
                 float b = fmaxf(fmaxf(s.st[0][1][n][0], s.st[0][1][n][1]), fmaxf(s.st[0][1][n][2], s.st[0][1][n][3]));
                 float c2 = fmaxf(fmaxf(s.st[1][0][n][0], s.st[1][0][n][1]), fmaxf(s.st[1][0][n][2], s.st[1][0][n][3]));
@@ -495,16 +547,17 @@
                 mx[n] = fmaxf(mx[n], fmaxf(fmaxf(a, b), fmaxf(c2, d2)));
             }
         };
-        auto set_reference = [&](const float (&mx)[4], float above) __attribute__((always_inline)) {
-#pragma unroll
-            for (int n = 0; n < 4; ++n) {
+        auto set_reference = [&](const float (&mx)[NQ], float above) __attribute__((always_inline)) {
+#pragma unroll
+            for (int n = 0; n < NQ; ++n) {
                 float m = fmaxf(mx[n], __shfl_xor(mx[n], 16, 64));
                 m = fmaxf(m, __shfl_xor(m, 32, 64)) + above;
                 s.mq[n] = (f32x4_t){-m, -m, -m, -m};
             }
         };
         if (attempt) {
-            float mx[4] = {-1e30f, -1e30f, -1e30f, -1e30f};
+            float mx[NQ] = {-1e30f, -1e30f, -1e30f, -1e30f};
+            if constexpr (NQ == 5) mx[4] = -1e30f;
 #pragma unroll
             for (int a = 0; a < 4; ++a) dma_k4(a, a);
             for (int t = 0; t < T; ++t) {
@@ -529,7 +582,8 @@
         bare_S(KB0{}, 0, 64);
         bare_S(KB1{}, 0, 64);
         if (attempt == 0) {
-            float mx[4] = {-1e30f, -1e30f, -1e30f, -1e30f};
+            float mx[NQ] = {-1e30f, -1e30f, -1e30f, -1e30f};
+            if constexpr (NQ == 5) mx[4] = -1e30f;
             tile_max(mx);
             set_reference(mx, c_log2 > 1e-20f ? 64.f / c_log2 : 0.f);
         }
@@ -538,12 +592,12 @@
 #pragma unroll
             for (int blk = 0; blk < 2; ++blk)
 #pragma unroll
-                for (int n = 0; n < 4; ++n) s.st[kb][blk][n] += s.mq[n];
+                for (int n = 0; n < NQ; ++n) s.st[kb][blk][n] += s.mq[n];
         m16_softmax_zero<0>(s, c_log2);
 #pragma unroll
-        for (int n = 0; n < 4; ++n) asm volatile("" : "+v"(s.l_run[n]));
+        for (int n = 0; n < NQ; ++n) asm volatile("" : "+v"(s.l_run[n]));
         prefetch(k_addr(1, 0), v_addr(0, 0));
-        m16_step<0, 1, true, true, SCALED, ORD>(s, qf, kf, vf, k_addr(1, 0), v_addr(0, 0), k_addr(1, 1), v_addr(0, 1), c_log2, M16NoDma());
+        m16_step<0, 1, true, true, SCALED, ORD, NQ>(s, qf, kf, vf, k_addr(1, 0), v_addr(0, 0), k_addr(1, 1), v_addr(0, 1), c_log2, M16NoDma());
         int t = 1;
         unsigned ka0 = k_addr(0, 0), ka1 = k_addr(1, 0), ka2 = k_addr(2, 0);
         unsigned va0 = v_addr(0, 0), va1 = v_addr(1, 0), va2 = v_addr(2, 0);
@@ -565,7 +619,7 @@
             const unsigned long long c0 = PROF ? __builtin_amdgcn_s_memtime() : 0;
             fence_hot();
             const unsigned long long c1 = PROF ? __builtin_amdgcn_s_memtime() : 0;
-            m16_step<1, 1, true, true, SCALED, ORD, 512, 8192, 0, 0>(s, qf, kf, vf, ka1, va0, ka2, va1, c_log2,
+            m16_step<1, 1, true, true, SCALED, ORD, NQ, 512, 8192, 0, 0>(s, qf, kf, vf, ka1, va0, ka2, va1, c_log2,
                                        [&](int n) __attribute__((always_inline)) {
                                            switch (n) {
                                                case 0: M16_BDMA0(dvo, rs_k, offk, lk0, 0); break;
@@ -579,7 +633,7 @@
                                            }
                                        });
             const unsigned long long c2 = PROF ? __builtin_amdgcn_s_memtime() : 0;
-            m16_step<0, 1, true, true, SCALED, ORD, 0, 0, 512, 8192>(s, qf, kf, vf, ka2, va1, ka2, va1, c_log2,
+            m16_step<0, 1, true, true, SCALED, ORD, NQ, 0, 0, 512, 8192>(s, qf, kf, vf, ka2, va1, ka2, va1, c_log2,
                                        [&](int n) __attribute__((always_inline)) {
                                            if (n == 0)
                                                asm volatile("s_add_u32 %0, %0, 0x4000\n\ts_add_u32 %1, %1, 0x4000" : "+s"(offk), "+s"(offv) : : "scc");
@@ -612,23 +666,23 @@
         if (t + 1 < T) {
             dma_v4(t + 1, s2);
         }
-        m16_step<1, 1, true, true, SCALED, ORD>(s, qf, kf, vf, k_addr(s1, 1), v_addr(s0, 1), k_addr(s2, 0), v_addr(s1, 0), c_log2, M16NoDma());
+        m16_step<1, 1, true, true, SCALED, ORD, NQ>(s, qf, kf, vf, k_addr(s1, 1), v_addr(s0, 1), k_addr(s2, 0), v_addr(s1, 0), c_log2, M16NoDma());
         if (t + 1 < T) {
             m16_mask_init<0>(s, last_lim, G, s.mq);
-            m16_step<0, 2, true, true, SCALED, ORD>(s, qf, kf, vf, k_addr(s2, 0), v_addr(s1, 0), k_addr(s2, 1), v_addr(s1, 1), c_log2, M16NoDma());
+            m16_step<0, 2, true, true, SCALED, ORD, NQ>(s, qf, kf, vf, k_addr(s2, 0), v_addr(s1, 0), k_addr(s2, 1), v_addr(s1, 1), c_log2, M16NoDma());
             fence();
             m16_mask_init<1>(s, last_lim, G, s.mq);
-            m16_step<1, 2, true, true, SCALED, ORD>(s, qf, kf, vf, k_addr(s2, 1), v_addr(s1, 1), k_addr(s2, 1), v_addr(s2, 0), c_log2, M16NoDma());
-            m16_step<0, 0, true, true, SCALED, ORD>(s, qf, kf, vf, k_addr(s2, 1), v_addr(s2, 0), k_addr(s2, 1), v_addr(s2, 1), c_log2, M16NoDma());
-            m16_step<1, 0, true, false, SCALED, ORD>(s, qf, kf, vf, k_addr(s2, 1), v_addr(s2, 1), k_addr(s2, 1), v_addr(s2, 1), c_log2, M16NoDma());
+            m16_step<1, 2, true, true, SCALED, ORD, NQ>(s, qf, kf, vf, k_addr(s2, 1), v_addr(s1, 1), k_addr(s2, 1), v_addr(s2, 0), c_log2, M16NoDma());
+            m16_step<0, 0, true, true, SCALED, ORD, NQ>(s, qf, kf, vf, k_addr(s2, 1), v_addr(s2, 0), k_addr(s2, 1), v_addr(s2, 1), c_log2, M16NoDma());
+            m16_step<1, 0, true, false, SCALED, ORD, NQ>(s, qf, kf, vf, k_addr(s2, 1), v_addr(s2, 1), k_addr(s2, 1), v_addr(s2, 1), c_log2, M16NoDma());
         } else {
-            m16_step<0, 0, true, true, SCALED, ORD>(s, qf, kf, vf, k_addr(s1, 1), v_addr(s1, 0), k_addr(s1, 1), v_addr(s1, 1), c_log2, M16NoDma());
-            m16_step<1, 0, true, false, SCALED, ORD>(s, qf, kf, vf, k_addr(s1, 1), v_addr(s1, 1), k_addr(s1, 1), v_addr(s1, 1), c_log2, M16NoDma());
+            m16_step<0, 0, true, true, SCALED, ORD, NQ>(s, qf, kf, vf, k_addr(s1, 1), v_addr(s1, 0), k_addr(s1, 1), v_addr(s1, 1), c_log2, M16NoDma());
+            m16_step<1, 0, true, false, SCALED, ORD, NQ>(s, qf, kf, vf, k_addr(s1, 1), v_addr(s1, 1), k_addr(s1, 1), v_addr(s1, 1), c_log2, M16NoDma());
         }
         m16_wait<0>();
         asm volatile("" ::"v"(kf[0]), "v"(kf[1]), "v"(kf[2]), "v"(kf[3]), "v"(vf[0]), "v"(vf[1]), "v"(vf[2]), "v"(vf[3]));
 #pragma unroll
-        for (int n = 0; n < 4; ++n) {
+        for (int n = 0; n < NQ; ++n) {
             s.l_run[n] += s.psa[n] + s.psb[n];
             s.psa[n] = s.psb[n] = 0.f;
             float lt = s.l_run[n] + __shfl_xor(s.l_run[n], 16, 64);
@@ -668,11 +722,11 @@
         qi = l3 & 15, G = l3 >> 4;
     }
 #pragma unroll
-    for (int n = 0; n < 4; ++n) {
+    for (int n = 0; n < NQ; ++n) {
         float l_tot = s.l_run[n] + __shfl_xor(s.l_run[n], 16, 64);
         l_tot += __shfl_xor(l_tot, 32, 64);
         const float inv = 1.f / l_tot;
-        const int64_t qr = (int64_t)qb0 * M16_QB + wave * 64 + n * 16 + qi;
+        const int64_t qr = (int64_t)qb0 * (64 * NQ) + wave * (16 * NQ) + n * 16 + qi;
         if (lse && G == 0 && qr < Lq) lse[(int64_t)head * Lq + qr] = (s.m_run[n] * c_log2 + __log2f(l_tot)) * 0.6931471805599453f;
         if (qr < Lq) {
             uint16_t* op = o + qr * ldo + head * 128 + G * 4;
@@ -715,20 +769,52 @@
 static unsigned* g_m16_flagcnt = nullptr;
 void mg_attn_m16_hooks(int dbg, unsigned long long* prof, unsigned* flagcnt) { g_m16_dbg = dbg, g_m16_prof = prof, g_m16_flagcnt = flagcnt; }
 
+static double m16_launch_cost(int64_t items, int n_cu, int item_q) {
+    if (items <= n_cu) return item_q;
+    if (items >= 32 * (int64_t)n_cu) return (double)items / n_cu * item_q;
+    const int64_t per = n_cu >= 8 ? n_cu / 8 : 1;
+    int64_t rounds = 0;
+    for (int x = 0; x < 8; ++x) {
+        const int64_t r = ((x + 1) * items / 8 - x * items / 8 + per - 1) / per;
+        rounds = r > rounds ? r : rounds;
+    }
+    return (double)rounds * item_q;
+}
+extern "C" int mg_attn_hd128_item_queries(int64_t Lq, int64_t Lk, int heads, int prescaled, int n_cu) {
+    if (!prescaled || n_cu < 8 || heads <= 0 || Lq <= 0 || Lk < 65520) return 256;
+    const int64_t items4 = (Lq + 255) / 256 * heads, items5 = (Lq + 319) / 320 * heads;
+    if (items4 < 6 * (int64_t)n_cu) return 256;
+    return 0.97 * m16_launch_cost(items5, n_cu, 320) < m16_launch_cost(items4, n_cu, 256) ? 320 : 256;
+}
+
 int mg_attn_m16_launch(const uint16_t* q, int64_t ldq, const uint16_t* kp, const uint16_t* vp, uint16_t* o, int64_t ldo,
-                       int64_t Lq, int64_t Lk, int heads, float c_log2, int prescaled, int nqb, float* lse, int reserve_cus,
+                       int64_t Lq, int64_t Lk, int heads, float c_log2, int prescaled, float* lse, int reserve_cus,
                        unsigned* workspace, hipStream_t st) {
     const int n_cu = mg_persistent_cus(reserve_cus);
     if (n_cu < 0) return MG_ERR_LAUNCH;
+    int item_q = mg_attn_hd128_item_queries(Lq, Lk, heads, prescaled, n_cu);
+#ifdef MG_AB_BUILD
+    if ((g_m16_dbg & 128) && prescaled) item_q = 320;
+    if (g_m16_dbg & 256) item_q = 256;
+#endif
+    const int64_t nqb64 = (Lq + item_q - 1) / item_q;
+    if (nqb64 * heads > 0x7fffffffLL) return MG_ERR_SHAPE;
+    const int nqb = (int)nqb64;
     const int total = nqb * heads;
     const unsigned grid = total <= n_cu ? (unsigned)total : (unsigned)n_cu;
     unsigned* tickets = nullptr;
     if (workspace && (int64_t)total >= 32 * (int64_t)grid && !(g_m16_dbg & 16))
         tickets = workspace;
 #define M16_ORD 9
-#define M16_LAUNCH(PROF, SCALED, ORD)                                                                                             \
-    hipLaunchKernelGGL((attn_hd128_m16_kernel<PROF, SCALED, ORD>), dim3(grid), dim3(M16_THREADS), 0, st, q, ldq, kp, vp, o, ldo, Lq, \
+#define M16_LAUNCH_NQ(PROF, SCALED, ORD, NQ)                                                                                      \
+    hipLaunchKernelGGL((attn_hd128_m16_kernel<PROF, SCALED, ORD, NQ>), dim3(grid), dim3(M16_THREADS), 0, st, q, ldq, kp, vp, o, ldo, Lq, \
                        Lk, heads, prescaled ? 1.0f : c_log2, nqb, g_m16_dbg, PROF ? g_m16_prof : nullptr, lse, g_m16_flagcnt, tickets)
+#define M16_LAUNCH(PROF, SCALED, ORD) M16_LAUNCH_NQ(PROF, SCALED, ORD, 4)
+    if (item_q == 320) {
+        if (g_m16_prof) M16_LAUNCH_NQ(true, false, M16_ORD, 5);
+        else M16_LAUNCH_NQ(false, false, M16_ORD, 5);
+        return mg_check_launch();
+    }
 #ifdef MG_AB_BUILD
     const int ord = (g_m16_dbg >> 1) & 7;
     const int mo = (g_m16_dbg >> 5) & 3;
@@ -756,5 +842,6 @@
         else M16_LAUNCH(false, true, M16_ORD);
     }
 #undef M16_LAUNCH
+#undef M16_LAUNCH_NQ
     return mg_check_launch();
 }
diff --git a/moviigen1.1_amd/wan/backend/lib.py b/moviigen1.1_amd/wan/backend/lib.py
--- a/moviigen1.1_amd/wan/backend/lib.py
+++ b/moviigen1.1_amd/wan/backend/lib.py
@@ -25,6 +25,7 @@
     'mg_gemm_mxfp8_gelu_q': [c_vp, c_i64, c_vp, c_i64, c_vp, c_i64, c_vp, c_i64, c_vp, c_i64, c_int, c_int, c_vp, c_i64, c_vp, c_i64,
                              c_vp],
     'mg_attn_workspace_bytes': [],
+    'mg_attn_hd128_item_queries': [c_i64, c_i64, c_int, c_int, c_int],
     'mg_attn_fwd_bf16_hd128': [c_vp, c_i64, c_vp, c_vp, c_vp, c_i64, c_i64, c_i64, c_int, c_f32, c_vp, c_vp],
     'mg_attn_fwd_bf16_hd128_lse': [c_vp, c_i64, c_vp, c_vp, c_vp, c_i64, c_vp, c_i64, c_i64, c_int, c_f32, c_vp, c_vp],
     'mg_attn_fwd_bf16_hd128_prescaled': [c_vp, c_i64, c_vp, c_vp, c_vp, c_i64, c_vp, c_i64, c_i64, c_int, c_int, c_vp, c_vp],
diff --git a/moviigen1.1_amd/wan/backend/ops.py b/moviigen1.1_amd/wan/backend/ops.py
--- a/moviigen1.1_amd/wan/backend/ops.py
+++ b/moviigen1.1_amd/wan/backend/ops.py
@@ -181,6 +181,10 @@
             ws = torch.zeros(int(lib.load().mg_attn_workspace_bytes()), dtype=torch.uint8, device=f'cuda:{dev}')
         _ATTN_WS[key] = ws
     return ws
+
+
+def attention_item_queries(lq, lk, heads, prescaled=True, n_cu=256):
+    return int(lib.load().mg_attn_hd128_item_queries(int(lq), int(lk), int(heads), int(bool(prescaled)), int(n_cu)))
 
 
 def attention_hd128(q, kp, vp, out, lk, heads, scale, prescaled=False, reserve_cus=0, workspace='stream', lse=None):
diff --git a/moviigen1.1_amd/wan/distributed/ulysses.py b/moviigen1.1_amd/wan/distributed/ulysses.py
--- a/moviigen1.1_amd/wan/distributed/ulysses.py
+++ b/moviigen1.1_amd/wan/distributed/ulysses.py
@@ -20,6 +20,8 @@
 
 
 def attention_rounds(n_heads, L, n_cu=256, qblock=256):
+    if qblock is None:
+        qblock = ops.attention_item_queries(L, L, n_heads, True, n_cu)
     items = n_heads * ((L + qblock - 1) // qblock)
     per_xcd_wg = max(1, (n_cu & ~7) // 8)
     if items <= (n_cu & ~7):
@@ -33,8 +35,11 @@
     t_exch = 4.0 * (L / P) * dim * 2 / P / (link_gbps * 1e9) * 1e3 if P > 1 else 0.0
     best = None
     for G in range(1, max(1, min(int(n_loc), int(max_groups))) + 1):
-        rounds = sum(attention_rounds(n, L, n_cu) for _, n in split_heads(n_loc, G))
-        cost = rounds * t_item + t_exch / G
+        rounds, cost = 0, t_exch / G
+        for _, n in split_heads(n_loc, G):
+            qb = ops.attention_item_queries(L, L, n, True, n_cu)
+            r = attention_rounds(n, L, n_cu, qb)
+            rounds, cost = rounds + r, cost + r * t_item * qb / 256
         if best is None or cost < best[2] - 1e-9 or (abs(cost - best[2]) <= 1e-9 and G > best[0]):
             best = (G, rounds, cost)
     return best
@@ -88,7 +93,7 @@
             self.peer = peer_copy.open_windows(group, self.recv + self.orecv)
         self.comm = torch.cuda.Stream(device=device)
         self.reserve_cus = 0 if self.peer is not None or len(self.groups) < 2 else int(os.environ.get('MOVIIGEN_SP_RESERVE_CUS', '0') or 0)
-        self.rounds = sum(attention_rounds(n, P * Lloc, (n_cu & ~7) - ((self.reserve_cus + 7) & ~7)) for _, n in self.groups)
+        self.rounds = sum(attention_rounds(n, P * Lloc, (n_cu & ~7) - ((self.reserve_cus + 7) & ~7), None if head_dim == 128 else 256) for _, n in self.groups)
         ev = lambda: [torch.cuda.Event() for _ in self.groups]
         self.ev_pack, self.ev_recv, self.ev_attn, self.ev_o = ev(), ev(), ev(), ev()
 
```
